# nagadomi/nunif

Hardware: AMD Instinct MI355X
Metric: input MPix/s, waifu2x swin_unet 2x tiled render (tile 256) of 1080p frames (higher is better)
Workload: dtype f16; 1 GPU; waifu2x swin_unet 2x (art scale2x geometry), tile_size=256, 1080p frame, random-init weights; tile_size=256, tile_batch=45, tiles_per_frame=45, concurrent_streams=2, parallelism=frame-sharded x1

## Files before the change

include/nunif_hip.h:

```cpp
#ifndef NUNIF_HIP_H
#define NUNIF_HIP_H

#include <stddef.h>
#include <stdint.h>

#ifdef __cplusplus
extern "C" {
#endif

#define NUNIF_HIP_ABI_VERSION 1

typedef enum {
    NUNIF_HIP_OK = 0,
    NUNIF_HIP_EINVAL = -1,
    NUNIF_HIP_ENOMEM = -2,
    NUNIF_HIP_EHIP = -3,
    NUNIF_HIP_EMISSING = -4,
    NUNIF_HIP_EUNSUPPORTED = -5
} nunif_hip_status;

int nunif_hip_abi_version(void);
const char *nunif_hip_last_error(void);

typedef struct {
    int32_t x_h, x_w, scale, offset, tile_size, blend_size;
    int32_t y_h, y_w, h_blocks, w_blocks;
    int32_t pad_l, pad_r, pad_t, pad_b, y_buffer_h, y_buffer_w;
    int32_t input_tile_step, output_tile_step;
    int32_t out_tile_size;
} nunif_tile_grid;

int nunif_hip_tile_grid_init(int32_t x_h, int32_t x_w, int32_t scale, int32_t offset, int32_t tile_size,
                             int32_t blend_size, nunif_tile_grid *grid);

int nunif_hip_blend_ramp(int32_t blend_size, float *ramp );

int nunif_hip_gather_tiles(const float *x, float *tiles, const nunif_tile_grid *grid, int32_t channels,
                           int32_t tile_begin, int32_t n_tiles, void *stream);

int nunif_hip_stitch_tiles(const float *tile_out, float *y, const nunif_tile_grid *grid, int32_t channels,
                           void *stream);

typedef struct {
    const char *name;
    const float *data;
    int32_t ndim;
    int64_t shape[4];
} nunif_tensor_desc;

typedef struct nunif_swin_unet nunif_swin_unet;

int nunif_hip_swin_unet_create(const nunif_tensor_desc *tensors, int32_t n_tensors, int32_t scale_factor,
                               nunif_swin_unet **handle);
void nunif_hip_swin_unet_destroy(nunif_swin_unet *handle);

int nunif_hip_swin_unet_forward(nunif_swin_unet *handle, const float *x, float *z, int32_t batch,
                                int32_t tile_size, void *stream);

int nunif_hip_swin_unet_render(nunif_swin_unet *handle, const float *x, float *y, int32_t x_h, int32_t x_w,
                               int32_t tile_size, int32_t batch_size, void *stream);

int nunif_hip_swin_unet_render_tile_rows(nunif_swin_unet *handle, const float *x, int32_t x_h, int32_t x_w,
                                         int32_t tile_size, int32_t batch_size, int32_t row_begin, int32_t row_end,
                                         void *stream);
int nunif_hip_swin_unet_tile_row_band(nunif_swin_unet *handle, int32_t x_h, int32_t x_w, int32_t tile_size,
                                      int32_t tile_row, int32_t row0, int32_t n_rows, float *band, int32_t import_band,
                                      void *stream);
int nunif_hip_swin_unet_stitch_rows(nunif_swin_unet *handle, float *y_band, int32_t x_h, int32_t x_w, int32_t tile_size,
                                    int32_t y_row_begin, int32_t y_row_end, void *stream);

typedef struct nunif_swin_unet_v2 nunif_swin_unet_v2;
int nunif_hip_swin_unet_v2_create(const nunif_tensor_desc *tensors, int32_t n_tensors, int32_t scale_factor,
                                  nunif_swin_unet_v2 **handle);
void nunif_hip_swin_unet_v2_destroy(nunif_swin_unet_v2 *handle);
int nunif_hip_swin_unet_v2_forward(nunif_swin_unet_v2 *handle, const float *x, float *z, int32_t batch, int32_t tile_size,
                                   int32_t clamp01, void *stream);

typedef struct nunif_cunet nunif_cunet;
int nunif_hip_cunet_create(const nunif_tensor_desc *tensors, int32_t n_tensors, int32_t no_clip, nunif_cunet **handle);
void nunif_hip_cunet_destroy(nunif_cunet *handle);
int nunif_hip_cunet_forward(nunif_cunet *handle, const float *x, float *z, int32_t batch, int32_t tile_size,
                            void *stream);
int nunif_hip_cunet_render(nunif_cunet *handle, const float *x, float *y, int32_t x_h, int32_t x_w,
                           int32_t tile_size, int32_t batch_size, void *stream);

int nunif_hip_tta_view(const float *x, float *y, int32_t C, int32_t H, int32_t W, int32_t view, void *stream);
int nunif_hip_tta_merge(const float *const *views, float *out, int32_t C, int32_t H, int32_t W, void *stream);
int nunif_hip_alpha_border_padding(const float *rgb, const float *alpha, float *out, float *work, int32_t H, int32_t W,
                                   int32_t offset, void *stream);

typedef struct {
    int32_t B, H, W;
    double divergence;
    double convergence;
    int32_t fill;
    int32_t synthetic_view;
    int32_t width_base;
    const float *convergence_dev;
} nunif_forward_warp_params;

int nunif_hip_forward_warp(const float *c, const float *depth, float *left, float *right, float *lmask,
                           float *rmask, const nunif_forward_warp_params *params, void *stream);

typedef struct nunif_depth_anything nunif_depth_anything;
int nunif_hip_depth_anything_create(const nunif_tensor_desc *tensors, int32_t n_tensors, nunif_depth_anything **handle);
int nunif_hip_depth_anything_create_ex(const nunif_tensor_desc *tensors, int32_t n_tensors, const int32_t *taps, float max_depth,
                                       nunif_depth_anything **handle);
void nunif_hip_depth_anything_destroy(nunif_depth_anything *handle);
int nunif_hip_depth_anything_forward(nunif_depth_anything *handle, const float *x, const float *pos, float *depth,
                                     int32_t B, int32_t h, int32_t w, void *stream);
int nunif_hip_depth_anything_reset_state(nunif_depth_anything *handle);
int nunif_hip_depth_anything_is_temporal(const nunif_depth_anything *handle);

typedef struct nunif_depth_aa nunif_depth_aa;
int nunif_hip_depth_aa_create(const nunif_tensor_desc *tensors, int32_t n_tensors, nunif_depth_aa **handle);
void nunif_hip_depth_aa_destroy(nunif_depth_aa *handle);
int nunif_hip_depth_aa_forward(nunif_depth_aa *handle, const float *x, float *y, int32_t B, int32_t h, int32_t w,
                               int32_t mode, void *stream);

typedef struct nunif_row_flow nunif_row_flow;
int nunif_hip_row_flow_create(const nunif_tensor_desc *tensors, int32_t n_tensors, nunif_row_flow **handle);
void nunif_hip_row_flow_destroy(nunif_row_flow *handle);
int nunif_hip_row_flow_delta(nunif_row_flow *handle, const float *x, float *delta, int32_t B, int32_t h, int32_t w,
                             int32_t flip, void *stream);

int nunif_hip_delta_warp(const float *c, const float *delta, float *out, int32_t B, int32_t C, int32_t H, int32_t W,
                         int32_t dh, int32_t dw, double delta_scale, int32_t flip, void *stream);

typedef struct nunif_light_inpaint nunif_light_inpaint;
int nunif_hip_light_inpaint_create(const nunif_tensor_desc *tensors, int32_t n_tensors, nunif_light_inpaint **handle);
void nunif_hip_light_inpaint_destroy(nunif_light_inpaint *handle);
int nunif_hip_light_inpaint_infer(nunif_light_inpaint *handle, const float *x, const uint8_t *mask, float *out, int32_t B,
                                  int32_t H, int32_t W, int32_t closing, int32_t inner_iter, int32_t outer_iter, void *stream);
int nunif_hip_light_inpaint_infer_ex(nunif_light_inpaint *handle, const float *x, const uint8_t *mask, float *out, int32_t B,
                                     int32_t H, int32_t W, int32_t closing, int32_t inner_iter, int32_t outer_iter,
                                     int32_t mirror_x, void *stream);

int nunif_hip_anaglyph(const float *left, const float *right, float *out, int32_t H, int32_t W, int32_t mode, void *stream);
int nunif_hip_equirectangular(const float *c, float *out, int32_t C, int32_t h, int32_t w, void *stream);

typedef struct nunif_mlbw nunif_mlbw;
int nunif_hip_mlbw_create(const nunif_tensor_desc *tensors, int32_t n_tensors, nunif_mlbw **handle);
void nunif_hip_mlbw_destroy(nunif_mlbw *handle);
int32_t nunif_hip_mlbw_num_layers(const nunif_mlbw *handle);
int nunif_hip_mlbw_delta(nunif_mlbw *handle, const float *x, float *delta, float *weight, int32_t B, int32_t h, int32_t w,
                         int32_t flip, void *stream);
int32_t nunif_hip_mlbw_has_hole_mask(const nunif_mlbw *handle);
int nunif_hip_mlbw_delta_mask(nunif_mlbw *handle, const float *x, float *delta, float *weight, float *mask_logits, int32_t B,
                              int32_t h, int32_t w, int32_t flip, void *stream);
int nunif_hip_hole_mask_postprocess(const float *logits, uint8_t *mask, float *work, int32_t B, int32_t h, int32_t w,
                                    int32_t H, int32_t W, float threshold, int32_t inner_iter, int32_t outer_iter, float *z,
                                    int32_t C, void *stream);

int nunif_hip_delta_weight_warp(const float *c, const float *delta, const float *weight, float *out, int32_t B, int32_t C,
                                int32_t H, int32_t W, int32_t dh, int32_t dw, int32_t L, double delta_scale, int32_t flip,
                                void *stream);

int nunif_hip_backward_warp(const float *c, const float *depth, float *left, float *right, int32_t B, int32_t C,
                            int32_t H, int32_t W, int32_t dh, int32_t dw, double divergence, double convergence,
                            int32_t synthetic_view, void *stream, const float *convergence_dev);

int nunif_hip_resize_aa(const float *x, float *y, float *tmp, int64_t planes, int32_t h_in, int32_t w_in,
                        int32_t h_out, int32_t w_out, int32_t bicubic, int32_t align_corners, int32_t clamp01,
                        const float *mean3, const float *std3, void *stream);

int64_t nunif_hip_dilate_edge_work_floats(int32_t B, int32_t H, int32_t W);
int nunif_hip_dilate_edge(const float *x, float *y, float *work, int32_t B, int32_t H, int32_t W, int32_t n_x,
                          int32_t n_y, void *stream);

int nunif_hip_minmax_normalize(const float *x, float *y, float *minmax, int32_t B, int64_t n_per, void *stream);

int nunif_hip_minmax(const float *x, float *minmax_keys, int32_t B, int64_t n_per, void *stream);
int nunif_hip_ema_scaler_push(float *state, const float *minmax_keys, int32_t ring_size, int64_t count, int32_t filled,
                              int32_t first, double decay, void *stream);
int nunif_hip_ema_scaler_ring_minmax(float *state, int32_t ring_size, void *stream);
int nunif_hip_range_normalize(const float *x, float *y, const float *lohi, int64_t n, int32_t max_mode, void *stream);

int nunif_hip_make_input_planes(const float *depth, float *out, int32_t B, int32_t H, int32_t W, double divergence_value,
                                double convergence_value, int32_t border_pix, void *stream, const float *convergence_dev);

int nunif_hip_stack(const void *const *srcs, int32_t n, int64_t bytes_each, void *dst, void *stream);

int nunif_hip_mask_morphology(const float *in, float *out, float *work, int32_t B, int32_t H, int32_t W, int32_t op,
                              int32_t n_a, int32_t n_b, void *stream);

int nunif_hip_reflection_pad2d(const float *x, float *y, int64_t planes, int32_t H, int32_t W, int32_t left, int32_t right,
                               int32_t top, int32_t bottom, void *stream);
int nunif_hip_depth_postprocess(const float *x, float *y, int64_t n, float max_dist, int32_t to_disparity, float eps,
                                int32_t negate, void *stream);

int nunif_hip_frame_to_tensor(const void *frame, float *chw, int32_t H, int32_t W, int32_t bits, void *stream);
int nunif_hip_stereo_to_frame(const float *left, const float *right, void *frame, int32_t H, int32_t W,
                              int32_t layout, int32_t bits, void *stream);
int nunif_hip_stereo_compose(const float *left, const float *right, float *out, int32_t H, int32_t W,
                             int32_t layout, void *stream);

int nunif_hip_rgb_noise(float *out, int32_t planes, int32_t H, int32_t W, int32_t level, int32_t component, uint64_t seed,
                        uint64_t counter, void *stream);
int nunif_hip_apply_rgb_noise(const float *rgb, const float *noise, float *out, int64_t n, double strength, double gamma,
                              int32_t light_decay, double light_decay_strength, void *stream);
int nunif_hip_grain_blend(float *buf, const float *noise, int64_t n, double speed, int32_t first, void *stream);
int nunif_hip_grain_video_step(const float *rgb, float *noise_buffer, void *frame, int32_t H, int32_t W, int32_t bits,
                               int32_t level, uint64_t seed, uint64_t counter, double speed, int32_t first, double strength,
                               double gamma, int32_t light_decay, double light_decay_strength, void *stream);
int nunif_hip_frame_to_tensor_rot(const void *frame, float *chw, int32_t H, int32_t W, int32_t bits, int32_t turns,
                                  void *stream);

int nunif_hip_map_depth(const float *x, float *y, int64_t n, int32_t kind, double p0, double p1, void *stream);

typedef struct nunif_transnetv2 nunif_transnetv2;
int nunif_hip_transnetv2_create(const nunif_tensor_desc *tensors, int32_t n_tensors, int32_t filters,
                                nunif_transnetv2 **handle);
void nunif_hip_transnetv2_destroy(nunif_transnetv2 *handle);
int nunif_hip_transnetv2_forward(nunif_transnetv2 *handle, const float *frames, int32_t B, int32_t T, float *one_hot,
                                 float *many_hot, float *sigmoid_out, void *stream);

typedef struct nunif_sod_v1 nunif_sod_v1;
int nunif_hip_sod_v1_create(const nunif_tensor_desc *tensors, int32_t n_tensors, int32_t net_size, nunif_sod_v1 **handle);
void nunif_hip_sod_v1_destroy(nunif_sod_v1 *handle);
int64_t nunif_hip_sod_v1_workspace_floats(int32_t B);
int nunif_hip_sod_v1_forward(nunif_sod_v1 *handle, const float *rgb, int32_t H, int32_t W, const float *depth, int32_t h,
                             int32_t w, int32_t B, float *workspace, float *saliency, float *depth_scaled, void *stream);
int nunif_hip_sod_v1_entry(const float *rgb, int32_t H, int32_t W, const float *depth, int32_t h, int32_t w, int32_t B,
                           float *x6, float *depth_scaled, void *stream);
int nunif_hip_sod_v1_debug_taps(nunif_sod_v1 *handle, const float *workspace, int32_t B, const char *name, float *out,
                                int64_t capacity, int64_t *shape4, void *stream);
int nunif_hip_sod_v1_depth_position(const float *saliency, const float *depth, int32_t B, int64_t n, double pos, float *out,
                                    void *stream);
int nunif_hip_sod_v1_ema(const float *z, float *out, int32_t B, float *state, double decay, uint64_t reset_mask, void *stream);

typedef struct nunif_superpoint nunif_superpoint;
int nunif_hip_superpoint_create(const nunif_tensor_desc *tensors, int32_t n_tensors, nunif_superpoint **handle);
void nunif_hip_superpoint_destroy(nunif_superpoint *handle);
int nunif_hip_superpoint_forward(nunif_superpoint *handle, const float *image, int32_t B, int32_t C, int32_t H, int32_t W,
                                 int32_t nms_radius, int32_t remove_borders, float threshold, float *keypoints,
                                 float *kp_scores, int32_t *counts, void *stream);
int nunif_hip_superpoint_debug_taps(nunif_superpoint *handle, const char *name, float *out, int64_t capacity, int64_t *shape4,
                                    void *stream);
int nunif_hip_superpoint_sample(nunif_superpoint *handle, int32_t b, const float *keypoints, int32_t n, float *out,
                                void *stream);

int64_t nunif_hip_superpoint_keypoints_work_floats(int32_t B, int32_t H, int32_t W);
int nunif_hip_superpoint_keypoints(const float *scores, int32_t B, int32_t H, int32_t W, int32_t nms_radius,
                                   int32_t remove_borders, float threshold, float *work, float *nms_out, float *keypoints,
                                   float *kp_scores, int32_t *counts, void *stream);

int nunif_hip_sample_descriptors(const float *keypoints, int32_t n, const float *dense, int32_t h, int32_t w, int32_t C,
                                 int32_t stride, float *out, void *stream);

int nunif_hip_superpoint_match(const float *d1, int32_t n1, const float *d2, int32_t n2, int32_t D, void *work, int64_t *index,
                               float *max_similarity, void *stream);

int nunif_hip_affine_warp(const float *x, const float *params, float *out, int32_t B, int32_t C, int32_t H, int32_t W,
                          int32_t padding_mode, void *stream);

typedef struct nunif_outpaint nunif_outpaint;
int nunif_hip_outpaint_create(const nunif_tensor_desc *tensors, int32_t n_tensors, nunif_outpaint **handle);
void nunif_hip_outpaint_destroy(nunif_outpaint *handle);
int64_t nunif_hip_outpaint_work_bytes(int32_t B, int32_t H, int32_t W, int32_t max_size);
int nunif_hip_outpaint_infer(nunif_outpaint *handle, const float *x, const uint8_t *mask, int32_t B, int32_t H, int32_t W,
                             int32_t max_size, int32_t mode, float *out, void *work, void *stream);
int nunif_hip_outpaint_debug_taps(nunif_outpaint *handle, const void *work, int32_t B, int32_t H, int32_t W, int32_t max_size,
                                  const char *name, float *out, int64_t capacity, int64_t *shape4, void *stream);
int nunif_hip_outpaint_buffer_step(const float *frames, const float *coarse, float *buffer, const uint8_t *reset,
                                   double buffer_decay, int32_t B, int32_t H, int32_t W, float *out, uint8_t *mask0,
                                   void *stream);

int nunif_hip_autocrop_stats(const float *x, int32_t B, int32_t H, int32_t W, int32_t flat, int32_t passes,
                             int32_t *border_count_tb, int32_t *border_count_lr, void *work, int64_t work_bytes, void *stream);
int nunif_hip_autocrop_debug_stats(const float *x, int32_t B, int32_t H, int32_t W, int32_t flat, int32_t passes,
                                   int32_t *border_count_tb, int32_t *border_count_lr, void *work, int64_t work_bytes,
                                   float *row_a, float *row_b, float *col_a, float *col_b, void *stream);
int nunif_hip_autocrop_crop_pad(const float *src, float *dst, int64_t N, int32_t sH, int32_t sW, int32_t dH, int32_t dW,
                                int32_t y0, int32_t x0, int32_t pad_top, int32_t pad_left, int32_t win_h, int32_t win_w,
                                float pad_value, void *stream);

int nunif_hip_jpeg_quant_tables(int32_t quality, uint8_t *luma, uint8_t *chroma);
int64_t nunif_hip_jpeg_header(int32_t H, int32_t W, int32_t quality, int32_t subsampling, int32_t restart_mcus, uint8_t *out,
                              int64_t capacity);
int64_t nunif_hip_jpeg_max_bytes(int32_t H, int32_t W, int32_t subsampling, int32_t restart_mcus);
int64_t nunif_hip_jpeg_workspace_bytes(int32_t B, int32_t H, int32_t W, int32_t subsampling, int32_t restart_mcus);
int nunif_hip_jpeg_encode(const float *rgb, int32_t B, int32_t H, int32_t W, int32_t quality, int32_t subsampling,
                          int32_t restart_mcus, uint8_t *out, int64_t capacity, int32_t *out_len, void *workspace, void *stream);
int nunif_hip_jpeg_debug_coefficients(const float *rgb, int32_t B, int32_t H, int32_t W, int32_t quality, int32_t subsampling,
                                      int16_t *coef, void *stream);

typedef struct nunif_hdr2sdr_params {
    double exposure, white_point, saturation_gain;
} nunif_hdr2sdr_params;
int nunif_hip_hdr2sdr(const void *src, void *dst, int32_t H, int32_t W, int32_t trc, int32_t colorspace,
                      const nunif_hdr2sdr_params *params, int32_t form, void *stream);
int nunif_hip_hdr2sdr_constants(int32_t trc, int32_t colorspace, const nunif_hdr2sdr_params *params, float *matrix,
                                float *hable_white);

typedef struct nunif_pixfmt_planes {
    void *data[3];
    int64_t pitch[3];
} nunif_pixfmt_planes;
int nunif_hip_yuv_to_tensor(const nunif_pixfmt_planes *src, int32_t format, int32_t H, int32_t W, int32_t matrix,
                            int32_t full_range, int32_t form, float *dst, void *frame, void *stream);
int nunif_hip_tensor_to_yuv(const float *src, int32_t H, int32_t W, int32_t format, int32_t matrix, int32_t full_range,
                            const nunif_pixfmt_planes *dst, void *stream);
int nunif_hip_pixfmt_constants(int32_t matrix, int32_t full_range, int32_t bits, int32_t direction, float *coefficients,
                               float *offsets);

typedef struct nunif_cliqa nunif_cliqa;
int nunif_hip_cliqa_create(const nunif_tensor_desc *tensors, int32_t n_tensors, int32_t kind, nunif_cliqa **handle);
void nunif_hip_cliqa_destroy(nunif_cliqa *handle);
int64_t nunif_hip_cliqa_workspace_bytes(nunif_cliqa *handle, int32_t B, int32_t H, int32_t W, int32_t group);
int nunif_hip_cliqa_forward(nunif_cliqa *handle, const float *x, int32_t B, int32_t H, int32_t W, int32_t group, void *workspace,
                            int64_t workspace_bytes, float *out0, float *out1, void *stream);
int nunif_hip_cliqa_debug_taps(nunif_cliqa *handle, const float *x, int32_t B, int32_t H, int32_t W, int32_t group,
                               void *workspace, int64_t workspace_bytes, float *out0, float *out1, void *tap1, void *tap2,
                               void *tap3, float *head_maps, void *stream);
int nunif_hip_cliqa_select_patches(const float *image, int32_t H, int32_t W, int32_t patch_size, int32_t num_patches,
                                   float *scores, int64_t *indices, float *patches, void *stream);

int64_t nunif_hip_png_header(int32_t H, int32_t W, int32_t form, const char *const *text_keys, const char *const *text_values,
                             int32_t n_text, uint8_t *out, int64_t capacity);
int64_t nunif_hip_png_max_bytes(int32_t H, int32_t W, int32_t form, int32_t stripe_rows);
int64_t nunif_hip_png_workspace_bytes(int32_t B, int32_t H, int32_t W, int32_t form, int32_t stripe_rows);
int nunif_hip_png_encode(const void *src, int32_t form, int32_t B, int32_t H, int32_t W, int32_t stripe_rows, uint8_t *out,
                         int64_t capacity, int32_t *out_len, void *workspace, void *stream);
int nunif_hip_png_debug_filtered(const void *src, int32_t form, int32_t B, int32_t H, int32_t W, uint8_t *filtered, void *stream);
int nunif_hip_png_debug_codes(const void *src, int32_t form, int32_t B, int32_t H, int32_t W, int32_t stripe_rows, int32_t *hist,
                              int32_t *lengths, void *workspace, void *stream);

int nunif_hip_swin_unet_debug_taps(nunif_swin_unet *handle, int32_t enable);
int nunif_hip_swin_unet_get_tap(nunif_swin_unet *handle, int32_t index, char *name, int32_t name_cap,
                                void *host_dst, int64_t cap_bytes, int64_t *nbytes);
int nunif_hip_cunet_debug_taps(nunif_cunet *handle, int32_t enable);
int nunif_hip_cunet_get_tap(nunif_cunet *handle, int32_t index, char *name, int32_t name_cap,
                            void *host_dst, int64_t cap_bytes, int64_t *nbytes);

int nunif_hip_profile_enable(int32_t on);
typedef struct { char name[48]; double total_ms; int64_t launches; double flops; double bytes; } nunif_prof_record;
int nunif_hip_profile_read(nunif_prof_record *out, int32_t cap, int32_t reset);

#ifdef __cplusplus
}
#endif
#endif
```

nunif_amd/_hip.py:

```python
import ctypes
import os

_HERE = os.path.dirname(os.path.abspath(__file__))
LIB_PATH = os.environ.get("NUNIF_HIP_LIB") or os.path.join(_HERE, "libnunif_hip.so")

c_void_p, c_int32, c_int64, c_float, c_char_p, c_double, c_uint64 = (
    ctypes.c_void_p, ctypes.c_int32, ctypes.c_int64, ctypes.c_float, ctypes.c_char_p, ctypes.c_double, ctypes.c_uint64)


class NunifHipError(RuntimeError):
    def __init__(self, status, message):
        super().__init__(f"libnunif_hip error {status}: {message}")
        self.status = status


class TileGrid(ctypes.Structure):
    _fields_ = [(n, c_int32) for n in (
        "x_h", "x_w", "scale", "offset", "tile_size", "blend_size",
        "y_h", "y_w", "h_blocks", "w_blocks",
        "pad_l", "pad_r", "pad_t", "pad_b", "y_buffer_h", "y_buffer_w",
        "input_tile_step", "output_tile_step", "out_tile_size")]

    def as_config(self):
        return {"y_h": self.y_h, "y_w": self.y_w, "h_blocks": self.h_blocks, "w_blocks": self.w_blocks,
                "pad": (self.pad_l, self.pad_r, self.pad_t, self.pad_b),
                "y_buffer_h": self.y_buffer_h, "y_buffer_w": self.y_buffer_w,
                "input_tile_step": self.input_tile_step, "output_tile_step": self.output_tile_step}


class TensorDesc(ctypes.Structure):
    _fields_ = [("name", c_char_p), ("data", c_void_p), ("ndim", c_int32), ("shape", c_int64 * 4)]


class ForwardWarpParams(ctypes.Structure):
    _fields_ = [("B", c_int32), ("H", c_int32), ("W", c_int32), ("divergence", c_double), ("convergence", c_double),
                ("fill", c_int32), ("synthetic_view", c_int32), ("width_base", c_int32), ("convergence_dev", c_void_p)]


class Hdr2SdrParams(ctypes.Structure):
    _fields_ = [("exposure", c_double), ("white_point", c_double), ("saturation_gain", c_double)]


class PixfmtPlanes(ctypes.Structure):
    _fields_ = [("data", c_void_p * 3), ("pitch", c_int64 * 3)]


class ProfRecord(ctypes.Structure):
    _fields_ = [("name", ctypes.c_char * 48), ("total_ms", c_double), ("launches", c_int64),
                ("flops", c_double), ("bytes", c_double)]


SIGNATURES = {
    "nunif_hip_abi_version": (c_int32, []),
    "nunif_hip_last_error": (c_char_p, []),
    "nunif_hip_tile_grid_init": (c_int32, [c_int32] * 6 + [ctypes.POINTER(TileGrid)]),
    "nunif_hip_blend_ramp": (c_int32, [c_int32, ctypes.POINTER(c_float)]),
    "nunif_hip_gather_tiles": (c_int32, [c_void_p, c_void_p, ctypes.POINTER(TileGrid), c_int32, c_int32, c_int32, c_void_p]),
    "nunif_hip_stitch_tiles": (c_int32, [c_void_p, c_void_p, ctypes.POINTER(TileGrid), c_int32, c_void_p]),
    "nunif_hip_swin_unet_create": (c_int32, [ctypes.POINTER(TensorDesc), c_int32, c_int32, ctypes.POINTER(c_void_p)]),
    "nunif_hip_swin_unet_destroy": (None, [c_void_p]),
    "nunif_hip_swin_unet_forward": (c_int32, [c_void_p, c_void_p, c_void_p, c_int32, c_int32, c_void_p]),
    "nunif_hip_swin_unet_render": (c_int32, [c_void_p, c_void_p, c_void_p, c_int32, c_int32, c_int32, c_int32, c_void_p]),
    "nunif_hip_swin_unet_render_tile_rows": (c_int32, [c_void_p, c_void_p, c_int32, c_int32, c_int32, c_int32, c_int32, c_int32, c_void_p]),
    "nunif_hip_swin_unet_tile_row_band": (c_int32, [c_void_p, c_int32, c_int32, c_int32, c_int32, c_int32, c_int32, c_void_p, c_int32, c_void_p]),
    "nunif_hip_swin_unet_stitch_rows": (c_int32, [c_void_p, c_void_p, c_int32, c_int32, c_int32, c_int32, c_int32, c_void_p]),
    "nunif_hip_swin_unet_v2_create": (c_int32, [ctypes.POINTER(TensorDesc), c_int32, c_int32, ctypes.POINTER(c_void_p)]),
    "nunif_hip_swin_unet_v2_destroy": (None, [c_void_p]),
    "nunif_hip_swin_unet_v2_forward": (c_int32, [c_void_p, c_void_p, c_void_p, c_int32, c_int32, c_int32, c_void_p]),
    "nunif_hip_cunet_create": (c_int32, [ctypes.POINTER(TensorDesc), c_int32, c_int32, ctypes.POINTER(c_void_p)]),
    "nunif_hip_cunet_destroy": (None, [c_void_p]),
    "nunif_hip_cunet_forward": (c_int32, [c_void_p, c_void_p, c_void_p, c_int32, c_int32, c_void_p]),
    "nunif_hip_cunet_render": (c_int32, [c_void_p, c_void_p, c_void_p, c_int32, c_int32, c_int32, c_int32, c_void_p]),
    "nunif_hip_forward_warp": (c_int32, [c_void_p, c_void_p, c_void_p, c_void_p, c_void_p, c_void_p,
                                         ctypes.POINTER(ForwardWarpParams), c_void_p]),
    "nunif_hip_backward_warp": (c_int32, [c_void_p, c_void_p, c_void_p, c_void_p] + [c_int32] * 6 +
                                [c_double, c_double, c_int32, c_void_p, c_void_p]),
    "nunif_hip_row_flow_create": (c_int32, [ctypes.POINTER(TensorDesc), c_int32, ctypes.POINTER(c_void_p)]),
    "nunif_hip_row_flow_destroy": (None, [c_void_p]),
    "nunif_hip_row_flow_delta": (c_int32, [c_void_p, c_void_p, c_void_p, c_int32, c_int32, c_int32, c_int32, c_void_p]),
    "nunif_hip_delta_warp": (c_int32, [c_void_p, c_void_p, c_void_p] + [c_int32] * 6 + [c_double, c_int32, c_void_p]),
    "nunif_hip_mlbw_create": (c_int32, [ctypes.POINTER(TensorDesc), c_int32, ctypes.POINTER(c_void_p)]),
    "nunif_hip_mlbw_destroy": (None, [c_void_p]),
    "nunif_hip_mlbw_num_layers": (c_int32, [c_void_p]),
    "nunif_hip_mlbw_delta": (c_int32, [c_void_p, c_void_p, c_void_p, c_void_p, c_int32, c_int32, c_int32, c_int32, c_void_p]),
    "nunif_hip_light_inpaint_create": (c_int32, [ctypes.POINTER(TensorDesc), c_int32, ctypes.POINTER(c_void_p)]),
    "nunif_hip_light_inpaint_destroy": (None, [c_void_p]),
    "nunif_hip_light_inpaint_infer": (c_int32, [c_void_p, c_void_p, c_void_p, c_void_p] + [c_int32] * 6 + [c_void_p]),
    "nunif_hip_light_inpaint_infer_ex": (c_int32, [c_void_p, c_void_p, c_void_p, c_void_p] + [c_int32] * 7 + [c_void_p]),
    "nunif_hip_anaglyph": (c_int32, [c_void_p, c_void_p, c_void_p, c_int32, c_int32, c_int32, c_void_p]),
    "nunif_hip_equirectangular": (c_int32, [c_void_p, c_void_p, c_int32, c_int32, c_int32, c_void_p]),
    "nunif_hip_mlbw_has_hole_mask": (c_int32, [c_void_p]),
    "nunif_hip_mlbw_delta_mask": (c_int32, [c_void_p, c_void_p, c_void_p, c_void_p, c_void_p, c_int32, c_int32, c_int32, c_int32,
                                            c_void_p]),
    "nunif_hip_hole_mask_postprocess": (c_int32, [c_void_p, c_void_p, c_void_p] + [c_int32] * 5 + [c_float, c_int32, c_int32,
                                                  c_void_p, c_int32, c_void_p]),
    "nunif_hip_delta_weight_warp": (c_int32, [c_void_p, c_void_p, c_void_p, c_void_p] + [c_int32] * 7 +
                                    [c_double, c_int32, c_void_p]),
    "nunif_hip_depth_aa_create": (c_int32, [ctypes.POINTER(TensorDesc), c_int32, ctypes.POINTER(c_void_p)]),
    "nunif_hip_depth_aa_destroy": (None, [c_void_p]),
    "nunif_hip_depth_aa_forward": (c_int32, [c_void_p, c_void_p, c_void_p, c_int32, c_int32, c_int32, c_int32, c_void_p]),
    "nunif_hip_depth_anything_create": (c_int32, [ctypes.POINTER(TensorDesc), c_int32, ctypes.POINTER(c_void_p)]),
    "nunif_hip_depth_anything_create_ex": (c_int32, [ctypes.POINTER(TensorDesc), c_int32, ctypes.POINTER(c_int32), ctypes.c_float,
                                                     ctypes.POINTER(c_void_p)]),
    "nunif_hip_depth_anything_destroy": (None, [c_void_p]),
    "nunif_hip_depth_anything_forward": (c_int32, [c_void_p, c_void_p, c_void_p, c_void_p, c_int32, c_int32, c_int32, c_void_p]),
    "nunif_hip_depth_anything_reset_state": (c_int32, [c_void_p]),
    "nunif_hip_depth_anything_is_temporal": (c_int32, [c_void_p]),
    "nunif_hip_tta_view": (c_int32, [c_void_p, c_void_p, c_int32, c_int32, c_int32, c_int32, c_void_p]),
    "nunif_hip_tta_merge": (c_int32, [ctypes.POINTER(c_void_p), c_void_p, c_int32, c_int32, c_int32, c_void_p]),
    "nunif_hip_alpha_border_padding": (c_int32, [c_void_p, c_void_p, c_void_p, c_void_p, c_int32, c_int32, c_int32, c_void_p]),
    "nunif_hip_resize_aa": (c_int32, [c_void_p, c_void_p, c_void_p, c_int64] + [c_int32] * 7 +
                            [ctypes.POINTER(c_float), ctypes.POINTER(c_float), c_void_p]),
    "nunif_hip_dilate_edge": (c_int32, [c_void_p, c_void_p, c_void_p] + [c_int32] * 5 + [c_void_p]),
    "nunif_hip_dilate_edge_work_floats": (ctypes.c_int64, [c_int32, c_int32, c_int32]),
    "nunif_hip_minmax_normalize": (c_int32, [c_void_p, c_void_p, c_void_p, c_int32, c_int64, c_void_p]),
    "nunif_hip_mask_morphology": (c_int32, [c_void_p, c_void_p, c_void_p] + [c_int32] * 6 + [c_void_p]),
    "nunif_hip_reflection_pad2d": (c_int32, [c_void_p, c_void_p, c_int64, c_int32, c_int32, c_int32, c_int32, c_int32, c_int32,
                                             c_void_p]),
    "nunif_hip_depth_postprocess": (c_int32, [c_void_p, c_void_p, c_int64, c_float, c_int32, c_float, c_int32, c_void_p]),
    "nunif_hip_frame_to_tensor": (c_int32, [c_void_p, c_void_p, c_int32, c_int32, c_int32, c_void_p]),
    "nunif_hip_stereo_to_frame": (c_int32, [c_void_p, c_void_p, c_void_p, c_int32, c_int32, c_int32, c_int32, c_void_p]),
    "nunif_hip_stereo_compose": (c_int32, [c_void_p, c_void_p, c_void_p, c_int32, c_int32, c_int32, c_void_p]),
    "nunif_hip_rgb_noise": (c_int32, [c_void_p, c_int32, c_int32, c_int32, c_int32, c_int32, c_uint64, c_uint64, c_void_p]),
    "nunif_hip_apply_rgb_noise": (c_int32, [c_void_p, c_void_p, c_void_p, c_int64, c_double, c_double, c_int32, c_double, c_void_p]),
    "nunif_hip_grain_blend": (c_int32, [c_void_p, c_void_p, c_int64, c_double, c_int32, c_void_p]),
    "nunif_hip_grain_video_step": (c_int32, [c_void_p, c_void_p, c_void_p, c_int32, c_int32, c_int32, c_int32, c_uint64, c_uint64,
                                             c_double, c_int32, c_double, c_double, c_int32, c_double, c_void_p]),
    "nunif_hip_frame_to_tensor_rot": (c_int32, [c_void_p, c_void_p, c_int32, c_int32, c_int32, c_int32, c_void_p]),
    "nunif_hip_map_depth": (c_int32, [c_void_p, c_void_p, c_int64, c_int32, c_double, c_double, c_void_p]),
    "nunif_hip_transnetv2_create": (c_int32, [ctypes.POINTER(TensorDesc), c_int32, c_int32, ctypes.POINTER(c_void_p)]),
    "nunif_hip_transnetv2_destroy": (None, [c_void_p]),
    "nunif_hip_transnetv2_forward": (c_int32, [c_void_p, c_void_p, c_int32, c_int32, c_void_p, c_void_p, c_void_p, c_void_p]),
    "nunif_hip_sod_v1_create": (c_int32, [ctypes.POINTER(TensorDesc), c_int32, c_int32, ctypes.POINTER(c_void_p)]),
    "nunif_hip_sod_v1_destroy": (None, [c_void_p]),
    "nunif_hip_sod_v1_workspace_floats": (c_int64, [c_int32]),
    "nunif_hip_sod_v1_forward": (c_int32, [c_void_p, c_void_p, c_int32, c_int32, c_void_p, c_int32, c_int32, c_int32, c_void_p,
                                           c_void_p, c_void_p, c_void_p]),
    "nunif_hip_sod_v1_entry": (c_int32, [c_void_p, c_int32, c_int32, c_void_p, c_int32, c_int32, c_int32, c_void_p, c_void_p,
                                         c_void_p]),
    "nunif_hip_sod_v1_debug_taps": (c_int32, [c_void_p, c_void_p, c_int32, c_char_p, c_void_p, c_int64, ctypes.POINTER(c_int64),
                                              c_void_p]),
    "nunif_hip_sod_v1_depth_position": (c_int32, [c_void_p, c_void_p, c_int32, c_int64, c_double, c_void_p, c_void_p]),
    "nunif_hip_sod_v1_ema": (c_int32, [c_void_p, c_void_p, c_int32, c_void_p, c_double, c_uint64, c_void_p]),
    "nunif_hip_superpoint_create": (c_int32, [ctypes.POINTER(TensorDesc), c_int32, ctypes.POINTER(c_void_p)]),
    "nunif_hip_superpoint_destroy": (None, [c_void_p]),
    "nunif_hip_superpoint_forward": (c_int32, [c_void_p, c_void_p] + [c_int32] * 6 + [c_float, c_void_p, c_void_p, c_void_p,
                                              c_void_p]),
    "nunif_hip_superpoint_debug_taps": (c_int32, [c_void_p, c_char_p, c_void_p, c_int64, ctypes.POINTER(c_int64), c_void_p]),
    "nunif_hip_superpoint_sample": (c_int32, [c_void_p, c_int32, c_void_p, c_int32, c_void_p, c_void_p]),
    "nunif_hip_superpoint_keypoints_work_floats": (c_int64, [c_int32, c_int32, c_int32]),
    "nunif_hip_superpoint_keypoints": (c_int32, [c_void_p] + [c_int32] * 5 + [c_float] + [c_void_p] * 6),
    "nunif_hip_sample_descriptors": (c_int32, [c_void_p, c_int32, c_void_p] + [c_int32] * 4 + [c_void_p, c_void_p]),
    "nunif_hip_superpoint_match": (c_int32, [c_void_p, c_int32, c_void_p, c_int32, c_int32, c_void_p, c_void_p, c_void_p,
                                            c_void_p]),
    "nunif_hip_affine_warp": (c_int32, [c_void_p, c_void_p, c_void_p] + [c_int32] * 5 + [c_void_p]),
    "nunif_hip_outpaint_create": (c_int32, [ctypes.POINTER(TensorDesc), c_int32, ctypes.POINTER(c_void_p)]),
    "nunif_hip_outpaint_destroy": (None, [c_void_p]),
    "nunif_hip_outpaint_work_bytes": (c_int64, [c_int32] * 4),
    "nunif_hip_outpaint_infer": (c_int32, [c_void_p, c_void_p, c_void_p] + [c_int32] * 5 + [c_void_p, c_void_p, c_void_p]),
    "nunif_hip_outpaint_debug_taps": (c_int32, [c_void_p, c_void_p] + [c_int32] * 4 + [c_char_p, c_void_p, c_int64,
                                                ctypes.POINTER(c_int64), c_void_p]),
    "nunif_hip_outpaint_buffer_step": (c_int32, [c_void_p] * 4 + [c_double] + [c_int32] * 3 + [c_void_p] * 3),
    "nunif_hip_autocrop_stats": (c_int32, [c_void_p] + [c_int32] * 5 + [c_void_p, c_void_p, c_void_p, c_int64, c_void_p]),
    "nunif_hip_autocrop_debug_stats": (c_int32, [c_void_p] + [c_int32] * 5 + [c_void_p, c_void_p, c_void_p, c_int64] +
                                       [c_void_p] * 5),
    "nunif_hip_autocrop_crop_pad": (c_int32, [c_void_p, c_void_p, c_int64] + [c_int32] * 10 + [c_float, c_void_p]),
    "nunif_hip_jpeg_quant_tables": (c_int32, [c_int32, c_void_p, c_void_p]),
    "nunif_hip_jpeg_header": (c_int64, [c_int32] * 5 + [c_void_p, c_int64]),
    "nunif_hip_jpeg_max_bytes": (c_int64, [c_int32] * 4),
    "nunif_hip_jpeg_workspace_bytes": (c_int64, [c_int32] * 5),
    "nunif_hip_jpeg_encode": (c_int32, [c_void_p] + [c_int32] * 6 + [c_void_p, c_int64, c_void_p, c_void_p, c_void_p]),
    "nunif_hip_jpeg_debug_coefficients": (c_int32, [c_void_p] + [c_int32] * 5 + [c_void_p, c_void_p]),
    "nunif_hip_png_header": (c_int64, [c_int32] * 3 + [c_void_p, c_void_p, c_int32, c_void_p, c_int64]),
    "nunif_hip_png_max_bytes": (c_int64, [c_int32] * 4),
    "nunif_hip_png_workspace_bytes": (c_int64, [c_int32] * 5),
    "nunif_hip_png_encode": (c_int32, [c_void_p] + [c_int32] * 5 + [c_void_p, c_int64, c_void_p, c_void_p, c_void_p]),
    "nunif_hip_png_debug_filtered": (c_int32, [c_void_p] + [c_int32] * 4 + [c_void_p, c_void_p]),
    "nunif_hip_png_debug_codes": (c_int32, [c_void_p] + [c_int32] * 5 + [c_void_p] * 4),
    "nunif_hip_hdr2sdr": (c_int32, [c_void_p, c_void_p, c_int32, c_int32, c_int32, c_int32, ctypes.POINTER(Hdr2SdrParams), c_int32,
                                    c_void_p]),
    "nunif_hip_hdr2sdr_constants": (c_int32, [c_int32, c_int32, ctypes.POINTER(Hdr2SdrParams), ctypes.POINTER(c_float),
                                              ctypes.POINTER(c_float)]),
    "nunif_hip_yuv_to_tensor": (c_int32, [ctypes.POINTER(PixfmtPlanes)] + [c_int32] * 6 + [c_void_p, c_void_p, c_void_p]),
    "nunif_hip_tensor_to_yuv": (c_int32, [c_void_p] + [c_int32] * 5 + [ctypes.POINTER(PixfmtPlanes), c_void_p]),
    "nunif_hip_pixfmt_constants": (c_int32, [c_int32] * 4 + [ctypes.POINTER(c_float), ctypes.POINTER(c_float)]),
    "nunif_hip_cliqa_create": (c_int32, [ctypes.POINTER(TensorDesc), c_int32, c_int32, ctypes.POINTER(c_void_p)]),
    "nunif_hip_cliqa_destroy": (None, [c_void_p]),
    "nunif_hip_cliqa_workspace_bytes": (c_int64, [c_void_p] + [c_int32] * 4),
    "nunif_hip_cliqa_forward": (c_int32, [c_void_p, c_void_p] + [c_int32] * 4 + [c_void_p, c_int64] + [c_void_p] * 3),
    "nunif_hip_cliqa_debug_taps": (c_int32, [c_void_p, c_void_p] + [c_int32] * 4 + [c_void_p, c_int64] + [c_void_p] * 7),
    "nunif_hip_cliqa_select_patches": (c_int32, [c_void_p] + [c_int32] * 4 + [c_void_p] * 4),
    "nunif_hip_swin_unet_debug_taps":(c_int32, [c_void_p, c_int32]),
    "nunif_hip_swin_unet_get_tap": (c_int32, [c_void_p, c_int32, c_char_p, c_int32, c_void_p, c_int64,
                                              ctypes.POINTER(c_int64)]),
    "nunif_hip_cunet_debug_taps": (c_int32, [c_void_p, c_int32]),
    "nunif_hip_cunet_get_tap": (c_int32, [c_void_p, c_int32, c_char_p, c_int32, c_void_p, c_int64,
                                          ctypes.POINTER(c_int64)]),
    "nunif_hip_minmax": (c_int32, [c_void_p, c_void_p, c_int32, c_int64, c_void_p]),
    "nunif_hip_ema_scaler_push": (c_int32, [c_void_p, c_void_p, c_int32, c_int64, c_int32, c_int32, c_double, c_void_p]),
    "nunif_hip_ema_scaler_ring_minmax": (c_int32, [c_void_p, c_int32, c_void_p]),
    "nunif_hip_range_normalize": (c_int32, [c_void_p, c_void_p, c_void_p, c_int64, c_int32, c_void_p]),
    "nunif_hip_make_input_planes": (c_int32, [c_void_p, c_void_p, c_int32, c_int32, c_int32, c_double, c_double, c_int32, c_void_p, c_void_p]),
    "nunif_hip_stack": (c_int32, [ctypes.POINTER(c_void_p), c_int32, c_int64, c_void_p, c_void_p]),
    "nunif_hip_profile_enable": (c_int32, [c_int32]),
    "nunif_hip_profile_read": (c_int32, [ctypes.POINTER(ProfRecord), c_int32, c_int32]),
}

_lib = None


def lib():
    global _lib
    if _lib is None:
        import torch
        if not os.path.exists(LIB_PATH):
            raise RuntimeError(
                f"{LIB_PATH} not found: the HIP engine is not built. Run `python -m nunif_amd.build` "
                "(there is no CPU fallback).")
        handle = ctypes.CDLL(LIB_PATH)
        for name, (restype, argtypes) in SIGNATURES.items():
            fn = getattr(handle, name)
            fn.restype = restype
            fn.argtypes = argtypes
        _lib = handle
    return _lib


def check(status):
    if status != 0:
        raise NunifHipError(status, lib().nunif_hip_last_error().decode("utf-8", "replace"))


def current_stream_ptr(device=None):
    import torch
    return c_void_p(torch.cuda.current_stream(device).cuda_stream)


def tile_grid(x_h, x_w, scale, offset, tile_size, blend_size):
    g = TileGrid()
    check(lib().nunif_hip_tile_grid_init(x_h, x_w, scale, offset, tile_size, blend_size or 0, ctypes.byref(g)))
    return g


def blend_ramp(blend_size):
    buf = (c_float * max(1, blend_size))()
    check(lib().nunif_hip_blend_ramp(blend_size, buf))
    return list(buf)[:blend_size]


def profile_enable(on=True):
    check(lib().nunif_hip_profile_enable(1 if on else 0))


def profile_read(reset=True):
    recs = (ProfRecord * 64)()
    n = lib().nunif_hip_profile_read(recs, 64, 1 if reset else 0)
    return [{"name": recs[i].name.decode(), "total_ms": recs[i].total_ms, "launches": recs[i].launches,
             "flops": recs[i].flops, "bytes": recs[i].bytes} for i in range(n)]
```

nunif_amd/csrc/swin_block_tail.hip:

```cpp
#include <algorithm>
#include <cstdlib>
#include <cstring>
#include <type_traits>

#include "swin_gelu.h"
#include "swin_kernels.h"

namespace nunif {

template <int C, int MF, int WAVES, bool PF = false, bool WM = false, bool G32 = false>
__global__ void __launch_bounds__(WAVES * 64)
proj_mlp_r_kernel(const f16 *__restrict__ att, f16 *x, const f16 *__restrict__ wstream, const float *__restrict__ bp,
                  const float *__restrict__ b0, const float *__restrict__ b3, long M, TailToImage ti, int rev, WinMap wm) {
    constexpr int KS = C / 32, NT = C / 16, SH = 2 * C / 32;
    constexpr int NF = 2 * KS * KS + SH * (2 * KS + NT);
    extern __shared__ __attribute__((aligned(16))) unsigned char smem_t[];
    f16x8 *wl = reinterpret_cast<f16x8 *>(smem_t);
    float *bl = reinterpret_cast<float *>(wl + (NF + KS) * 64);

    const int tid = threadIdx.x;
    const int lane = tid & 63;
    const int wave = tid >> 6;
    const int r16 = lane & 15;
    const int grp = lane >> 4;
    {
        const f16x8 *src = reinterpret_cast<const f16x8 *>(wstream);
        for (int i = tid; i < NF * 64; i += WAVES * 64) wl[i] = src[i];
        for (int i = tid; i < C; i += WAVES * 64) { bl[i] = bp[i]; bl[3 * C + i] = b3[i]; }
        for (int i = tid; i < 2 * C; i += WAVES * 64) bl[C + i] = b0[i];
        if (ti.w) {
            for (int i = tid; i < KS * 64; i += WAVES * 64) wl[NF * 64 + i] = reinterpret_cast<const f16x8 *>(ti.w)[i];
            if (tid < 16) bl[4 * C + tid] = tid < ti.n_real ? ti.bias[tid] : 0.f;
        }
    }
    __syncthreads();
    const f16x8 *wlane = wl + lane;
    auto wfrag = [&](int fi) -> f16x8 { return wlane[fi * 64]; };
    f16x8 ie, io, je, jo;
#pragma unroll
    for (int j = 0; j < 8; ++j) {
        ie[j] = (f16)((r16 == 8 * grp + j) ? 1.f : 0.f);
        io[j] = (f16)((r16 + 16 == 8 * grp + j) ? 1.f : 0.f);
        je[j] = (f16)((j < 4 && r16 == 4 * grp + j) ? 1.f : 0.f);
        jo[j] = (f16)((j >= 4 && r16 == 4 * grp + j - 4) ? 1.f : 0.f);
    }

    const long n_groups = (M + MF * 16 - 1) / (MF * 16);
    const long gstride = (long)gridDim.x * WAVES;
    auto gmap = [&](long g) { return rev ? n_groups - 1 - g : g; };
    auto token_of = [&](long g, int f) -> long {
        const long m = gmap(g) * (MF * 16) + f * 16 + r16;
        return m < M ? m : M - 1;
    };
    auto load_pixmap = [&](long g, int (&pm)[MF]) {
#pragma unroll
        for (int f = 0; f < MF; ++f) pm[f] = wm.pixmap[(int)token_of(g, f)];
    };
    auto load_group = [&](long g, const int (&pm)[MF], f16x8 (&of)[MF][KS], f16x8 (&xr)[MF][KS], long (&pixn)[MF]) {
#pragma unroll
        for (int f = 0; f < MF; ++f) {
            const long r = token_of(g, f);
            const f16 *p;
            if constexpr (WM) {
                const int ri = (int)r, w = ri / 36;
                pixn[f] = pm[f];
                p = att + (ri * 16 + w * 2880 + (grp >> 1) * 576 + 8 * (grp & 1));
            } else {
                pixn[f] = r;
                p = att + r * C + grp * 8;
            }
            const f16 *px = x + pixn[f] * C + grp * 8;
#pragma unroll
            for (int ks = 0; ks < KS; ++ks) {
                of[f][ks] = *reinterpret_cast<const f16x8 *>(p + (WM ? ks * (2 * 36 * 16) : ks * 32));
                xr[f][ks] = *reinterpret_cast<const f16x8 *>(px + ks * 32);
            }
        }
    };
    f16x8 ofn[PF ? MF : 1][PF ? KS : 1];
    f16x8 xrn[PF ? MF : 1][PF ? KS : 1];
    long pixnn[MF];
    const long g_first = (long)blockIdx.x * WAVES + wave;
    int pm_next[MF] = {};
    auto g_clamp = [&](long g) { return g < n_groups ? g : n_groups - 1; };
    if constexpr (PF) {
        if (g_first < n_groups) {
            if constexpr (WM) load_pixmap(g_first, pm_next);
            load_group(g_first, pm_next, ofn, xrn, pixnn);
            if constexpr (WM) load_pixmap(g_clamp(g_first + gstride), pm_next);
        }
    }
#pragma unroll 1
    for (long g = g_first; g < n_groups; g += gstride) {
        const long m_base = gmap(g) * (MF * 16);
        int lofs = 0;
        asm volatile("" : "+v"(lofs));
        const float *lbp = bl + lofs, *lb0 = bl + C + lofs, *lb3 = bl + 3 * C + lofs;
        long row[MF];
        bool valid[MF];
        f16x8 yf[MF][KS];
        {
            f16x8 of[MF][KS];
            f16x8 xr[MF][KS];
#pragma unroll
            for (int f = 0; f < MF; ++f) {
                const long m = m_base + f * 16 + r16;
                valid[f] = m < M;
            }
            if constexpr (PF) {
#pragma unroll
                for (int f = 0; f < MF; ++f) {
                    row[f] = pixnn[f];
#pragma unroll
                    for (int ks = 0; ks < KS; ++ks) { of[f][ks] = ofn[f][ks]; xr[f][ks] = xrn[f][ks]; }
                }
                load_group(g_clamp(g + gstride), pm_next, ofn, xrn, pixnn);
                if constexpr (WM) load_pixmap(g_clamp(g + 2 * gstride), pm_next);
            } else {
                if constexpr (WM) load_pixmap(g, pm_next);
                load_group(g, pm_next, of, xr, row);
            }
#pragma unroll
            for (int s = 0; s < KS; ++s) {
                const int n0 = 32 * s + 4 * grp;
                const f32x4 ba = *reinterpret_cast<const f32x4 *>(lbp + n0);
                const f32x4 bb = *reinterpret_cast<const f32x4 *>(lbp + n0 + 16);
                f32x4 a0[MF], a1[MF];
#pragma unroll
                for (int f = 0; f < MF; ++f) { a0[f] = ba; a1[f] = bb; }
#pragma unroll
                for (int ks = 0; ks < KS; ++ks) {
                    const f16x8 wa = wfrag((s * KS + ks) * 2);
                    const f16x8 wb = wfrag((s * KS + ks) * 2 + 1);
#pragma unroll
                    for (int f = 0; f < MF; ++f) {
                        a0[f] = MFMA_16x16x32(wa, of[f][ks], a0[f]);
                        a1[f] = MFMA_16x16x32(wb, of[f][ks], a1[f]);
                    }
                }
#pragma unroll
                for (int f = 0; f < MF; ++f) {
                    a0[f] = MFMA_16x16x32(ie, xr[f][s], a0[f]);
                    a1[f] = MFMA_16x16x32(io, xr[f][s], a1[f]);
                }
#pragma unroll
                for (int f = 0; f < MF; ++f)
                    yf[f][s] = (f16x8){(f16)a0[f][0], (f16)a0[f][1], (f16)a0[f][2], (f16)a0[f][3],
                                       (f16)a1[f][0], (f16)a1[f][1], (f16)a1[f][2], (f16)a1[f][3]};
            }
        }
        f32x4 acc[NT][MF];
#pragma unroll
        for (int s = 0; s < KS; ++s) {
            const int n0 = 32 * s + 4 * grp;
            const f32x4 ca = *reinterpret_cast<const f32x4 *>(lb3 + n0);
            const f32x4 cb = *reinterpret_cast<const f32x4 *>(lb3 + n0 + 16);
#pragma unroll
            for (int f = 0; f < MF; ++f) {
                acc[2 * s][f] = MFMA_16x16x32(je, yf[f][s], ca);
                acc[2 * s + 1][f] = MFMA_16x16x32(jo, yf[f][s], cb);
            }
        }
        constexpr int F_MLP = 2 * KS * KS;
        constexpr int F_STEP = 2 * KS + NT;
#pragma unroll 1
        for (int s = 0; s < SH; ++s) {
            const int n0 = 32 * s + 4 * grp;
            const f32x4 ba = *reinterpret_cast<const f32x4 *>(lb0 + n0);
            const f32x4 bb = *reinterpret_cast<const f32x4 *>(lb0 + n0 + 16);
            f32x4 h0[MF], h1[MF];
#pragma unroll
            for (int f = 0; f < MF; ++f) { h0[f] = ba; h1[f] = bb; }
            const f16x8 *wf = wlane + (F_MLP + s * F_STEP) * 64;
#pragma unroll
            for (int ks = 0; ks < KS; ++ks) {
                const f16x8 wa = wf[(ks * 2) * 64];
                const f16x8 wb = wf[(ks * 2 + 1) * 64];
#pragma unroll
                for (int f = 0; f < MF; ++f) {
                    h0[f] = MFMA_16x16x32(wa, yf[f][ks], h0[f]);
                    h1[f] = MFMA_16x16x32(wb, yf[f][ks], h1[f]);
                }
            }
            f16x8 hf[MF];
#pragma unroll
            for (int f = 0; f < MF; ++f) {
                hf[f] = gelu8t<G32>(h0[f], h1[f]);
            }
#pragma unroll
            for (int nt = 0; nt < NT; ++nt) {
                const f16x8 wv = wf[(2 * KS + nt) * 64];
#pragma unroll
                for (int f = 0; f < MF; ++f) acc[nt][f] = MFMA_16x16x32(wv, hf[f], acc[nt][f]);
            }
        }
        if (ti.w) {
            const int s2 = ti.ps * ti.ps;
            const f32x4 tb = *reinterpret_cast<const f32x4 *>(bl + 4 * C + 4 * grp);
#pragma unroll
            for (int f = 0; f < MF; ++f) {
                f32x4 img = tb;
#pragma unroll
                for (int ks = 0; ks < KS; ++ks) {
                    const f16x8 bfrag = {(f16)acc[2 * ks][f][0], (f16)acc[2 * ks][f][1], (f16)acc[2 * ks][f][2], (f16)acc[2 * ks][f][3],
                                         (f16)acc[2 * ks + 1][f][0], (f16)acc[2 * ks + 1][f][1], (f16)acc[2 * ks + 1][f][2],
                                         (f16)acc[2 * ks + 1][f][3]};
                    img = MFMA_16x16x32(wlane[(NF + ks) * 64], bfrag, img);
                }
                if (!valid[f]) continue;
                using pix_t = std::conditional_t<WM, unsigned, long>;
                const pix_t m = (pix_t)row[f];
                const int px = (int)(m % (pix_t)ti.W);
                const pix_t t2 = m / (pix_t)ti.W;
                const int py = (int)(t2 % (pix_t)ti.H), pb = (int)(t2 / (pix_t)ti.H);
                const int OC = ti.n_real / s2;
                const long OH = (long)ti.H * ti.ps, OW = (long)ti.W * ti.ps;
#pragma unroll
                for (int r = 0; r < 4; ++r) {
                    const int n = 4 * grp + r;
                    if (n < ti.n_real) {
                        const int c = n / s2, rem = n - c * s2, i = rem / ti.ps, j = rem - i * ti.ps;
                        ti.out[(((long)pb * OC + c) * OH + (long)py * ti.ps + i) * OW + (long)px * ti.ps + j] =
                            fminf(fmaxf(img[r], 0.f), 1.f);
                    }
                }
            }
            continue;
        }
#pragma unroll
        for (int p = 0; p < NT / 2; ++p) {
#pragma unroll
            for (int f = 0; f < MF; ++f) {
                const f16x4 oa = {(f16)acc[2 * p][f][0], (f16)acc[2 * p][f][1], (f16)acc[2 * p][f][2], (f16)acc[2 * p][f][3]};
                const f16x4 ob = {(f16)acc[2 * p + 1][f][0], (f16)acc[2 * p + 1][f][1], (f16)acc[2 * p + 1][f][2],
                                  (f16)acc[2 * p + 1][f][3]};
                const f16x8 o = pair_to_run(oa, ob);
                if (valid[f]) *reinterpret_cast<f16x8 *>(x + row[f] * C + 32 * p + pair_run_channel(grp)) = o;
            }
        }
    }
}

__global__ void winmap_build_kernel(int *__restrict__ pixmap, int B, int H, int W, int shift) {
    const int n = blockIdx.x * blockDim.x + threadIdx.x;
    const int nwx = W / 6, nwy = H / 6;
    if (n >= B * H * W) return;
    const int w = n / 36, t = n - 36 * w;
    const int wx = w % nwx, t2 = w / nwx;
    const int wy = t2 % nwy, b = t2 / nwy;
    const int iy = t / 6, ix = t - 6 * iy;
    int yy = wy * 6 + iy + shift, xx = wx * 6 + ix + shift;
    if (yy >= H) yy -= H;
    if (xx >= W) xx -= W;
    pixmap[n] = (b * H + yy) * W + xx;
}

int launch_winmap_build(int *pixmap, int B, int H, int W, int shift, hipStream_t s) {
    NUNIF_REQUIRE(H % 6 == 0 && W % 6 == 0 && (long)B * H * W < (1L << 31), "winmap: geometry %d x %d x %d", B, H, W);
    const long n = (long)B * H * W;
    if (n == 0) return NUNIF_HIP_OK;
    winmap_build_kernel<<<(unsigned)((n + 255) / 256), 256, 0, s>>>(pixmap, B, H, W, shift);
    NUNIF_LAUNCH_CHECK();
    return NUNIF_HIP_OK;
}

constexpr int proj_mlp_stream_frags_c(int C) { return 2 * (C / 32) * (C / 32) + (2 * C / 32) * (2 * (C / 32) + C / 16); }

int proj_mlp_stream_frags(int C) {
    const int KS = C / 32, NT = C / 16, SH = 2 * C / 32;
    return 2 * KS * KS + SH * (2 * KS + NT);
}

int launch_proj_mlp(const f16 *att, f16 *x, const f16 *wstream, const float *bp, const float *b0, const float *b3,
                    long M, int C, hipStream_t s, const TailToImage *to_image, int rev, const WinMap *wmap, int gelu32) {
    if (M == 0) return NUNIF_HIP_OK;
    NUNIF_REQUIRE(C == 96, "proj_mlp: channel count %d unsupported (C = 192 runs launch_proj_mlp_ws)", C);
    NUNIF_REQUIRE(!to_image || to_image->n_real <= 16, "proj_mlp: the fused image head takes at most 16 output channels");
    ProfScope ps("proj_mlp_r_kernel<96,2,8,true>", s, 2.0 * (double)M * C * C * 5.0, (double)M * C * 2.0 * 3.0);
    constexpr size_t smem = (size_t)(proj_mlp_stream_frags_c(96) + 3) * 1024 + (4 * 96 + 16) * 4;
    TailToImage ti;
    memset(&ti, 0, sizeof(ti));
    if (to_image) ti = *to_image;
    WinMap wm;
    memset(&wm, 0, sizeof(wm));
    if (wmap) wm = *wmap;
    NUNIF_REQUIRE(!wm.on || (wm.pixmap && wm.H % 6 == 0 && wm.W % 6 == 0 && M % ((long)wm.H * wm.W) == 0 && 96L * M < (1L << 31)),
                  "proj_mlp: window map geometry");
    constexpr int MF = 2, WAVES = 8;
    auto go = [&](auto kern, int slot) -> int {
        static bool configured[4] = {false, false, false, false};
        if (!configured[slot]) {
            NUNIF_HIP_CHECK(hipFuncSetAttribute((const void *)kern, hipFuncAttributeMaxDynamicSharedMemorySize, (int)smem));
            configured[slot] = true;
        }
        const long groups = (M + MF * 16 - 1) / (MF * 16);
        const unsigned blocks = (unsigned)std::min<long>((groups + WAVES - 1) / WAVES, 256);
        kern<<<blocks, WAVES * 64, smem, s>>>(att, x, wstream, bp, b0, b3, M, ti, rev, wm);
        return NUNIF_HIP_OK;
    };
    int rc;
    if (gelu32) rc = wm.on ? go(proj_mlp_r_kernel<96, MF, WAVES, true, true, true>, 3) : go(proj_mlp_r_kernel<96, MF, WAVES, true, false, true>, 2);
    else rc = wm.on ? go(proj_mlp_r_kernel<96, MF, WAVES, true, true, false>, 1) : go(proj_mlp_r_kernel<96, MF, WAVES, true, false, false>, 0);
    if (rc) return rc;
    NUNIF_LAUNCH_CHECK();
    return NUNIF_HIP_OK;
}

}
```

nunif_amd/csrc/swin_kernels.h:

```cpp
#pragma once
#include "common.h"

namespace nunif {

struct GemmArgs {
    const f16 *a; int B, Hi, Wi, Cin;
    int Ho, Wo, stride, oy, ox, kw;
    int K;
    const f16 *w;
    const float *bias;
    int N;
    int mode;
    int act;
    float slope;
    const f16 *res;
    void *out;
    int ldo;
    int n_real;
    int ps;
    int oshift, OH, OW;
    int no_clamp;
    int lda;
    int rev;
    int nt_chunk;
    int res_H = 0, res_W = 0, res_crop = 0;
    const float *in_scale = nullptr;
};
int launch_gemm(const GemmArgs &g, hipStream_t s, const char *tag);

struct PatchUpArgs { const f16 *a, *w; const float *bias; const f16 *res; f16 *out; int B, Ho, Wo, Cq, rev; };
bool patchup_supported(const PatchUpArgs &g);
int launch_patchup(const PatchUpArgs &g, hipStream_t s);

struct PatchDownArgs { const f16 *a, *w; const float *bias; f16 *out; int B, Ho, Wo, Cin, oy, rev; int N = 192; int act = 0; float slope = 0.f; };
bool patchdown_supported(const PatchDownArgs &g);
int launch_patchdown(const PatchDownArgs &g, hipStream_t s);

struct CunetUpArgs { const f16 *a, *w; const float *bias; const f16 *res; f16 *out; const float *in_scale; int B, S, res_S, crop;
                     float slope; };
bool cunet_up_supported(const CunetUpArgs &g);
int launch_cunet_up(const CunetUpArgs &g, hipStream_t s);

struct GemmOsArgs {
    const f16 *a; long M; int lda, K;
    const f16 *w; const float *bias; int N;
    int act;
    const f16 *res;
    f16 *out; int ldo;
    float2 *stats_out;
    const float2 *stats_in; int stats_parts; const float *wsum; float ln_eps;
};
bool gemm_os_supported(long M, int N, int K);
bool gemm_os_consumes_stats(long M, int N, int K);
int launch_gemm_os(const GemmOsArgs &g, hipStream_t s, const char *tag);

struct DaMlpArgs {
    f16 *t; long M;
    const f16 *w1; const float *b1, *ws1;
    const f16 *w2c; const float *b2;
    const float2 *stats_in; float2 *stats_out; float ln_eps;
    void *partial; unsigned *flags;
};
bool da_mlp_supported(int D, int hidden);

struct CunetHeadArgs { const f16 *a, *w; const float *bias; float *out32; const float *add32; int B, Hi, Wi, Ho, Wo, addH, addW, add_crop, clamp01; };
bool cunet_head_supported(const CunetHeadArgs &g);
int launch_cunet_head(const CunetHeadArgs &g, hipStream_t s);

constexpr int kVdaGnBlocks = 256;
int launch_vda_groupnorm(const f16 *x, const float *gamma, const float *beta, f16 *y, float2 *part, int frames, int P, int C, float eps, hipStream_t s);
int launch_vda_layernorm(const f16 *x, const float *gamma, const float *beta, f16 *y, long T, int C, float eps, hipStream_t s);
int launch_vda_geglu(const f16 *h, f16 *out, long T, int I, hipStream_t s);
struct VdaTattnArgs { const f16 *qkv; f16 *kc, *vc; const float *pq, *pk, *pv; f16 *att; int P, C, hd, start, idx; };
int launch_vda_tattn(const VdaTattnArgs &g, hipStream_t s);
long da_mlp_partial_bytes(long M);
long da_mlp_flag_count(long M);
int launch_da_mlp(const DaMlpArgs &a, hipStream_t s);

struct Stem1Args {
    const float *x;
    int frame_mode, H, W, wb, istep, pad_t, pad_l, tile_begin;
    int B, T;
    const float *w;
    const float *bias;
    int C1, C1P;
    f16 *out;
    float slope;
};
int launch_stem1(const Stem1Args &a, hipStream_t s);

struct StemFusedArgs {
    const float *x;
    int frame_mode, H, W, wb, istep, pad_t, pad_l, tile_begin;
    int B, T;
    const f16 *w1;
    const f16 *w2;
    const float *b2;
    f16 *out;
    float slope;
    int rev;
    int C1, C, crop;
};
bool stem_fused_supported(int C1, int C);
int launch_stem_fused(const StemFusedArgs &a, hipStream_t s);

int proj_mlp_stream_frags(int C);
struct TailToImage { const f16 *w; const float *bias; float *out; int H, W, ps, n_real; };
struct WinMap { int on, H, W, shift; const int *pixmap; };
int launch_winmap_build(int *pixmap, int B, int H, int W, int shift, hipStream_t s);
int launch_proj_mlp(const f16 *att, f16 *x, const f16 *wstream, const float *bp, const float *b0, const float *b3,
                    long M, int C, hipStream_t s, const TailToImage *to_image = nullptr, int rev = 0,
                    const WinMap *wm = nullptr, int gelu32 = 0);

int swin_block96_tail_frags();
int swin_block96_btab_floats();
int launch_swin_block96(f16 *x, const f16 *wqkv, const float *bqkv, const float *btab, const f16 *wtail, const float *bp,
                        const float *b0, const float *b3, int B, int H, int W, int shift, hipStream_t s,
                        const TailToImage *ti = nullptr, int rev = 0);

int proj_mlp_ws_stream_frags();
int launch_proj_mlp_ws(const f16 *att, f16 *x, const f16 *wws, const float *bp, const float *b0, const float *b3, long M,
                       hipStream_t s, int rev = 0, int gelu32 = 0);

constexpr int kQkvBiasFloatsPerHead = 36 * 52;
int launch_qkv_attn_r(const f16 *x, f16 *att, const f16 *wres, const float *bqkv, const float *btab32,
                      int B, int H, int W, int C, int heads, int shift, hipStream_t s, int rev = 0, int window_major = 0);

int launch_window_attn(const f16 *qkv, f16 *out, const float *bias, int B, int H, int W, int heads, int hd,
                       int shift, hipStream_t s);

int launch_layernorm_nobias(const f16 *x, f16 *y, const float *gamma, long M, int C, hipStream_t s);

struct ConvArgs {
    const f16 *a; const f16 *a2;
    int H2, W2, crop2;
    int B, Hi, Wi, Cin, Ho, Wo, stride, kh, kw;
    const f16 *wstream;
    const float *bias;
    int N, n_real;
    int act; float slope;
    f16 *out;
    float *out32;
    const float *add32; int addH, addW, add_crop;
    int clamp01;
    int rpad;
    const f16 *res;
    int zpad;
    int relu_in;
    const f16 *res2;
    int ldo;
    int cmaj;
    float *part32;
};
long gemm_big_m();
int launch_conv(const ConvArgs &g, hipStream_t s);
bool conv3_lds_applies(const ConvArgs &g);
int launch_conv3_lds(const ConvArgs &g, hipStream_t s);
bool conv3_dma_applies(const ConvArgs &g);
int launch_conv3_dma(const ConvArgs &g, hipStream_t s);

struct C3ConvArgs {
    const float *x; int frame_mode, H, W, wb, istep, pad_t, pad_l, tile_begin;
    int B, T;
    const float *w, *bias;
    int C;
    f16 *out;
    float slope;
};
int launch_c3_conv(const C3ConvArgs &a, hipStream_t s);

int launch_se(f16 *x, float *sums, float *scale, const float *w1, const float *b1, const float *w2, const float *b2,
              int B, long hw, int C, hipStream_t s, int scale_in_consumer = 0);

}
```

nunif_amd/csrc/swin_qkv_attn_r.hip:

```cpp
#include <algorithm>
#include <cstdlib>

#include "swin_kernels.h"

namespace nunif {


constexpr float kRegionR = 100.0f;

struct QkvAttnRArgs {
    const f16 *x;
    f16 *att;
    const f16 *wres;
    const float *bqkv;
    const float *btab32;
    int B, H, W, shift, n_windows;
    int rev;
};

__device__ __forceinline__ f16x4 mul4_to_f16(const f32x4 &o, float inv) {
    return (f16x4){(f16)__builtin_fmaf(o[0], inv, 0.0f), (f16)__builtin_fmaf(o[1], inv, 0.0f), (f16)__builtin_fmaf(o[2], inv, 0.0f),
                   (f16)__builtin_fmaf(o[3], inv, 0.0f)};
}
__device__ __forceinline__ f16x4 lone_to_f16x4(float e, float zf) {
    return (f16x4){(f16)e, (f16)zf, (f16)0.f, (f16)0.f};
}

constexpr int kBiasStride = 52;


__device__ __host__ inline int win_token(int mt, int r16) { return mt < 2 ? 16 * mt + r16 : ((r16 & 3) == 0 ? 32 + (r16 >> 2) : 35); }

template <int C, int HD, int HPP, int WAVES = 8, bool WM = false>
__global__ void __launch_bounds__(WAVES * 64)
qkv_attn_r_kernel(QkvAttnRArgs a) {
    constexpr int kWavesR = WAVES;
    constexpr int NTHR = WAVES * 64;
    constexpr int KS = C / 32;
    constexpr int HEADS = C / HD;
    constexpr int NTH = HD / 16;
    constexpr int FPH = 3 * NTH * KS;
    constexpr int PASSES = HEADS / HPP;
    static_assert(HEADS == 6 && HEADS % HPP == 0, "swin_unet uses 6 heads at every level");
    extern __shared__ __attribute__((aligned(16))) unsigned char smem_r[];
    f16x8 *wl = reinterpret_cast<f16x8 *>(smem_r);
    float *bt32 = reinterpret_cast<float *>(wl + HPP * FPH * 64);
    float *bl = bt32 + HPP * kQkvBiasFloatsPerHead;

    const int tid = threadIdx.x;
    const int lane = tid & 63;
    const int wave = __builtin_amdgcn_readfirstlane(tid >> 6);
    const int r16 = lane & 15;
    const int grp = lane >> 4;
    const int nwx = a.W / 6, nwy = a.H / 6;
    const f16x4 zero4 = {(f16)0.f, (f16)0.f, (f16)0.f, (f16)0.f};
    float zf = 0.f;
    asm("" : "+s"(zf));

    for (int i = tid; i < 3 * C; i += NTHR) bl[i] = a.bqkv[i];
    const f16x8 ones8 = {(f16)1.f, (f16)1.f, (f16)1.f, (f16)1.f, (f16)1.f, (f16)1.f, (f16)1.f, (f16)1.f};

    int tokc[3];
#pragma unroll
    for (int mt = 0; mt < 3; ++mt) tokc[mt] = win_token(mt, r16);
    unsigned wm_off[3];
#pragma unroll
    for (int mt = 0; mt < 3; ++mt) wm_off[mt] = (unsigned)((tokc[mt] * HD + 4 * grp) * 2);
    const bool store2 = (r16 & 3) == 0;
    const int st_delta = (NTH == 2 ? pair_run_channel(grp) : 4 * grp) * 2 - 16 * grp;
    f16x4 rk0 = zero4, rq0 = zero4;
    if (a.shift > 0 && grp == 2) { rk0[0] = (f16)1.f; rq0[0] = (f16)kRegionR; }

    const int n_wg = gridDim.x / PASSES;
    const int wstride = kWavesR * n_wg;
    const bool spread = a.n_windows < 8 * wstride;
    const int w0 = spread ? wave * n_wg + (int)(blockIdx.x / PASSES) : (int)(blockIdx.x / PASSES) * kWavesR + wave;
    const int pass = blockIdx.x % PASSES;
    {
        const f16x8 *src = reinterpret_cast<const f16x8 *>(a.wres) + (long)pass * HPP * FPH * 64;
        for (int i = tid; i < HPP * FPH * 64; i += NTHR) wl[i] = src[i];
        const f32x4 *bsrc = reinterpret_cast<const f32x4 *>(a.btab32 + (long)pass * HPP * kQkvBiasFloatsPerHead);
        for (int i = tid; i < HPP * kQkvBiasFloatsPerHead / 4; i += NTHR) reinterpret_cast<f32x4 *>(bt32)[i] = bsrc[i];
    }
    __syncthreads();

    int cx = w0 % nwx, cy = (w0 / nwx) % nwy, cb = w0 / (nwx * nwy);
    const int dx = wstride % nwx, dy = (wstride / nwx) % nwy, db = wstride / (nwx * nwy);
    const long img_bytes = (long)a.H * a.W * C * 2;

    auto load_x = [&](int wb, int wy, int wx, bool special, f16x8 (&xf)[3][KS], unsigned (&vo)[3]) {
        const int y0 = wy * 6 + a.shift, x0 = wx * 6 + a.shift;
        const char *xb = reinterpret_cast<const char *>(a.x) + (long)wb * img_bytes;
        if (special) {
#pragma unroll
            for (int mt = 0; mt < 3; ++mt) {
                const int tk = win_token(mt, r16), iy = tk / 6, ix = tk - 6 * iy;
                int yy = y0 + iy, xx = x0 + ix;
                if (yy >= a.H) yy -= a.H;
                if (xx >= a.W) xx -= a.W;
                vo[mt] = (unsigned)(((yy * a.W + xx) * C + 8 * grp) * 2);
            }
        } else {
            const unsigned org = (unsigned)((y0 * a.W + x0) * C * 2);
            int rl = r16;
            asm("" : "+v"(rl));
#pragma unroll
            for (int mt = 0; mt < 3; ++mt) {
                const int tk = win_token(mt, rl), iy = (tk * 43) >> 8, ix = tk - 6 * iy;
                vo[mt] = org + (unsigned)(((iy * a.W + ix) * C + 8 * grp) * 2);
            }
        }
#pragma unroll
        for (int mt = 0; mt < 3; ++mt) {
#pragma unroll
            for (int ks = 0; ks < KS; ++ks) xf[mt][ks] = *reinterpret_cast<const f16x8 *>(xb + vo[mt] + 64 * ks);
        }
    };
    auto decode = [&](int &wb, int &wy, int &wx, bool &special) {
        wb = a.rev ? a.B - 1 - cb : cb;
        wy = a.rev ? nwy - 1 - cy : cy;
        wx = a.rev ? nwx - 1 - cx : cx;
        special = a.shift > 0 && (wy == nwy - 1 || wx == nwx - 1);
    };
    auto advance = [&]() {
        cx += dx;
        if (cx >= nwx) { cx -= nwx; ++cy; }
        cy += dy;
        if (cy >= nwy) { cy -= nwy; ++cb; }
        cb += db;
    };

    auto qkv_bias = [&](int hl, int head, int part, int nt) -> f32x4 {
        const int ch0 = part * C + head * HD + nt * 16;
        if (part == 2) { const float bv = bl[ch0 + r16]; return (f32x4){bv, bv, bv, bv}; }
        return *reinterpret_cast<const f32x4 *>(bl + ch0 + 4 * grp);
    };
    auto bias_frag = [&](int hl, int qt, int kt) -> f32x4 {
        return *reinterpret_cast<const f32x4 *>(bt32 + (hl * 36 + tokc[qt]) * kBiasStride + 4 * grp + 16 * kt);
    };
    f16x8 xf[3][KS];
    unsigned vo[3];
    int wb, wy, wx;
    bool special;
    f16x8 wnx = wl[lane];
    auto run_windows = [&]() {
    int wi = w0;
    decode(wb, wy, wx, special);
    auto step = [&]() { advance(); wi += wstride; decode(wb, wy, wx, special); };
    if (wi < a.n_windows) load_x(wb, wy, wx, special, xf, vo);
#pragma unroll 1
    while (wi < a.n_windows) {
        const int wq = (wb * nwy + wy) * nwx + wx;
        char *ab = reinterpret_cast<char *>(a.att) + (WM ? (long)wq * (HEADS * 36 * HD * 2) : (long)wb * img_bytes);
        const unsigned wm_base = (unsigned)__builtin_amdgcn_readfirstlane((unsigned)wq * (unsigned)(HEADS * 36 * HD * 2));

        constexpr bool kEarlyX = C == 96 && WM;
        auto run_heads = [&]() {
        const bool sp_now = special;
        f16x4 rkr[3], rqr[3];
        if (special) {
            const bool last_y = wy == nwy - 1, last_x = wx == nwx - 1;
#pragma unroll
            for (int mt = 0; mt < 3; ++mt) {
                const int tk = win_token(mt, r16), iy = tk / 6, ix = tk - 6 * iy;
                const int reg = ((last_y && iy >= 3) ? 2 : 0) + ((last_x && ix >= 3) ? 1 : 0);
#pragma unroll
                for (int j = 0; j < 4; ++j) {
                    const bool on = grp == 2 && reg == j;
                    rkr[mt][j] = (f16)(on ? 1.f : 0.f);
                    rqr[mt][j] = (f16)(on ? kRegionR : 0.f);
                }
            }
        } else {
#pragma unroll
            for (int mt = 0; mt < 3; ++mt) { rkr[mt] = rk0; rqr[mt] = rq0; }
        }
        constexpr int kHeadUnroll = C == 96 ? HPP : 1;
#pragma unroll kHeadUnroll
        for (int hl = 0; hl < HPP; ++hl) {
            const int head = pass * HPP + hl;
            const f16x8 *wh = wl + (hl * FPH) * 64 + lane;
            constexpr bool kPrefetchW = C == 96;
            f16x4 qt4[NTH][3], kt4[NTH][3], vt4[NTH][3];
            f16x8 wq2[2];
            wq2[0] = kPrefetchW ? wnx : wh[0];
            f32x4 bnx = qkv_bias(hl, head, 0, 0);
#pragma unroll
            for (int part = 0; part < 3; ++part) {
#pragma unroll
                for (int nt = 0; nt < NTH; ++nt) {
                    const int fidx = (part * NTH + nt) * KS;
                    f32x4 acc[3];
                    bnx = qkv_bias(hl, head, part, nt);
#pragma unroll
                    for (int mt = 0; mt < 3; ++mt) acc[mt] = bnx;
#pragma unroll
                    for (int ks = 0; ks < KS; ++ks) {
                        const int f = fidx + ks;
                        if constexpr (kPrefetchW)
                            wq2[(f + 1) & 1] = (f + 1 < FPH) ? wh[(f + 1) * 64] : (hl + 1 < HPP ? wh[FPH * 64] : wl[lane]);
                        else wq2[f & 1] = wh[f * 64];
                        const f16x8 w = wq2[f & 1];
#pragma unroll
                        for (int mt = 0; mt < 3; ++mt)
                            acc[mt] = part == 2 ? MFMA_16x16x32(xf[mt][ks], w, acc[mt]) : MFMA_16x16x32(w, xf[mt][ks], acc[mt]);
                    }
#pragma unroll
                    for (int mt = 0; mt < 3; ++mt) {
                        const f16x4 v = {(f16)acc[mt][0], (f16)acc[mt][1], (f16)acc[mt][2], (f16)acc[mt][3]};
                        if (part == 0) qt4[nt][mt] = v; else if (part == 1) kt4[nt][mt] = v; else vt4[nt][mt] = v;
                    }
                }
            }
            if constexpr (kPrefetchW) wnx = wq2[FPH & 1];
            if constexpr (kEarlyX) {
                if (hl == HPP - 1) {
                    step();
                    if (wi < a.n_windows) load_x(wb, wy, wx, special, xf, vo);
                }
            }

#pragma unroll
            for (int qt = 0; qt < 3; ++qt) {
                f32x4 s[3];
                {
                    f32x4 sb[3];
#pragma unroll
                    for (int kt = 0; kt < 3; ++kt) sb[kt] = bias_frag(hl, qt, kt);
#pragma unroll
                    for (int kt = 0; kt < 3; ++kt) {
                        f32x4 acc = sb[kt];
                        if constexpr (HD == 16) {
                            acc = MFMA_16x16x32(cat8(kt4[0][kt], rkr[kt]), cat8(qt4[0][qt], rqr[qt]), acc);
                        } else {
                            acc = MFMA_16x16x32(cat8(kt4[0][kt], kt4[1][kt]), cat8(qt4[0][qt], qt4[1][qt]), acc);
                            if (sp_now) acc = MFMA_16x16x32(cat8(rkr[kt], zero4), cat8(rqr[qt], zero4), acc);
                        }
                        s[kt] = acc;
                    }
                }
                float mx = fmaxf(fmaxf(fmaxf(fmaxf(s[0][0], s[0][1]), s[0][2]), fmaxf(fmaxf(s[0][3], s[1][0]), s[1][1])),
                                 fmaxf(fmaxf(s[1][2], s[1][3]), s[2][0]));
                mx = row_group_max(mx);
                f16x4 pf[3];
#pragma unroll
                for (int kt = 0; kt < 2; ++kt) {
                    const float p0 = __builtin_amdgcn_exp2f(s[kt][0] - mx), p1 = __builtin_amdgcn_exp2f(s[kt][1] - mx);
                    const float p2 = __builtin_amdgcn_exp2f(s[kt][2] - mx), p3 = __builtin_amdgcn_exp2f(s[kt][3] - mx);
                    pf[kt] = (f16x4){(f16)p0, (f16)p1, (f16)p2, (f16)p3};
                }
                pf[2] = lone_to_f16x4(__builtin_amdgcn_exp2f(s[2][0] - mx), zf);
                const f16x8 psum = cat8(pf[0] + pf[1], pf[2]);
                const f32x4 z4 = {0.f, 0.f, 0.f, 0.f};
                const f32x4 sm = MFMA_16x16x32(ones8, psum, z4);
                const float inv = __builtin_amdgcn_rcpf(sm[0]);
                const bool store = qt < 2 || store2;
                f16x4 ov[NTH];
#pragma unroll
                for (int dt = 0; dt < NTH; ++dt) {
                    f32x4 o = MFMA_16x16x32(cat8(vt4[dt][0], vt4[dt][1]), cat8(pf[0], pf[1]), z4);
                    o = MFMA_16x16x32(cat8(zero4, vt4[dt][2]), psum, o);
                    ov[dt] = mul4_to_f16(o, inv);
                }
                if constexpr (NTH == 2) {
                    const f16x8 run = pair_to_run(ov[0], ov[1]);
                    if (store) *reinterpret_cast<f16x8 *>(ab + (vo[qt] + (unsigned)st_delta) + head * (HD * 2)) = run;
                } else if constexpr (WM) {
                    unsigned long hb = reinterpret_cast<unsigned long>(a.att) + (wm_base + (unsigned)(head * (36 * HD * 2)));
                    asm("" : "+s"(hb));
                    typedef __attribute__((address_space(1))) char gchar;
                    typedef __attribute__((address_space(1))) f16x4 gf16x4;
                    unsigned lo = wm_off[qt];
                    asm("" : "+v"(lo));
                    if (store) *reinterpret_cast<gf16x4 *>(reinterpret_cast<gchar *>(hb) + lo) = ov[0];
                } else {
                    if (store) *reinterpret_cast<f16x4 *>(ab + (vo[qt] + (unsigned)st_delta) + head * (HD * 2)) = ov[0];
                }
            }
            if constexpr (kHeadUnroll > 1) __builtin_amdgcn_sched_barrier(0);
        }
        };
        run_heads();

        if constexpr (!kEarlyX) {
            step();
            if (wi < a.n_windows) load_x(wb, wy, wx, special, xf, vo);
        }
    }
    };
    run_windows();
}

int qkv_attn_r_frags(int C) { return 3 * (C / 16) * (C / 32); }

template <int C, int HD, int HPP, int WAVES = 8, bool WM = false>
static int launch_r(const QkvAttnRArgs &a, int grid, hipStream_t s) {
    constexpr size_t smem = (size_t)HPP * 3 * (HD / 16) * (C / 32) * 1024 + HPP * kQkvBiasFloatsPerHead * 4 + (size_t)3 * C * 4;
    static bool configured = false;
    if (!configured) {
        NUNIF_HIP_CHECK(hipFuncSetAttribute((const void *)qkv_attn_r_kernel<C, HD, HPP, WAVES, WM>,
                                            hipFuncAttributeMaxDynamicSharedMemorySize, (int)smem));
        configured = true;
    }
    qkv_attn_r_kernel<C, HD, HPP, WAVES, WM><<<grid, WAVES * 64, smem, s>>>(a);
    return NUNIF_HIP_OK;
}

int launch_qkv_attn_r(const f16 *x, f16 *att, const f16 *wres, const float *bqkv, const float *btab32,
                      int B, int H, int W, int C, int heads, int shift, hipStream_t s, int rev, int window_major) {
    NUNIF_REQUIRE(H % 6 == 0 && W % 6 == 0, "qkv_attn: %dx%d not a multiple of the 6x6 window", H, W);
    NUNIF_REQUIRE(heads == 6 && (C == 96 || C == 192), "qkv_attn: C=%d heads=%d unsupported", C, heads);
    if (H <= 6) shift = 0;
    QkvAttnRArgs a;
    a.x = x; a.att = att; a.wres = wres; a.bqkv = bqkv; a.btab32 = btab32;
    a.B = B; a.H = H; a.W = W; a.shift = shift;
    a.n_windows = B * (H / 6) * (W / 6);
    a.rev = rev;
    NUNIF_REQUIRE(!window_major || C == 96, "qkv_attn: the window-major att map exists for C = 96 only");
    NUNIF_REQUIRE(!window_major || (long)a.n_windows * (6 * 36 * 16 * 2) < (1L << 32),
                  "qkv_attn: the window-major att map of %d windows does not fit 32-bit byte offsets", a.n_windows);
    const double tok = (double)B * H * W;
    const int kWavesR = C == 96 ? 16 : 8;
    const int wgs = (a.n_windows + kWavesR - 1) / kWavesR;
    int grid = wgs < 256 ? wgs : 256;
    if (C == 192) grid = std::max(2, grid & ~1);
    int rc;
    if (C == 96) {
        ProfScope ps("qkv_attn_r_kernel<96,16>", s, 2.0 * tok * C * 3.0 * C + 4.0 * tok * 36.0 * C, tok * C * 4.0);
        rc = window_major ? launch_r<96, 16, 6, 16, true>(a, grid, s) : launch_r<96, 16, 6, 16, false>(a, grid, s);
    } else {
        ProfScope ps("qkv_attn_r_kernel<192,32>", s, 2.0 * tok * C * 3.0 * C + 4.0 * tok * 36.0 * C, tok * C * 4.0);
        rc = launch_r<192, 32, 3>(a, grid, s);
    }
    if (rc) return rc;
    NUNIF_LAUNCH_CHECK();
    return NUNIF_HIP_OK;
}

}
```

nunif_amd/csrc/swin_unet.cpp:

```cpp
#include <algorithm>
#include <cmath>
#include <cstdlib>
#include <cstring>
#include <string>
#include <vector>

#include "host_weights.h"
#include "swin_kernels.h"

namespace nunif {

int launch_stitch(const float *tile_out, float *y, const nunif_tile_grid *g, int C, hipStream_t s, int y0 = 0, int rows = -1,
                  int compact = 0);

namespace {

struct Linear {
    f16 *w = nullptr;
    float *bias = nullptr;
    int N = 0, n_real = 0, K = 0;
};

struct Block {
    Linear qkv, proj, mlp0, mlp3;
    Linear mlp0p, mlp3p;
    float *norm1 = nullptr, *norm2 = nullptr;
    bool fast = true;
    float *attn_bias = nullptr;
    f16 *tail_stream = nullptr;
    f16 *tail_ws = nullptr;
    f16 *qkv_res = nullptr;
    float *qkv_rbias = nullptr;
    float *attn_btab32 = nullptr;
    f16 *b96_tail = nullptr;
    float *b96_btab = nullptr;
};

}
}

using namespace nunif;

struct nunif_swin_unet : DeviceOwner {
    int scale_factor = 2;
    int C = 96, heads = 6;
    int C1 = 48, C1P = 64;
    int top_dim = 96;
    float *stem1_w = nullptr, *stem1_b = nullptr;
    Linear stem2, down1, down2, up2, up1, proj2, to_image, to_image_pre;
    Linear down2b;
    bool down2_split = false;
    f16 *to_image_chained = nullptr;
    f16 *stemf_w1 = nullptr, *stemf_w2 = nullptr;
    int dir = 0;
    int att_wm = 1;
    int gelu32 = 0;
    int block96 = 0;
    bool has_proj2 = false;
    std::vector<Block> swin[5];
    DeviceBuf s1, f1, f2, f3, g1, qkv, att, hid, tile_out;
    DeviceBuf winmap[2];
    int winmap_B = 0, winmap_S = 0;
    int device = 0;
    struct Tap { std::string name; void *dev; size_t bytes; };
    bool taps_on = false;
    std::vector<Tap> taps;
    void clear_taps() { for (auto &t : taps) (void)hipFree(t.dev); taps.clear(); }
};

namespace nunif {
namespace {

int pad16(int n) { return (n + 15) / 16 * 16; }

template <typename F>
int make_linear(nunif_swin_unet *h, int n_real, int K, F wt, const float *bias, Linear *L, bool chained = false,
                std::vector<f16> *keep = nullptr) {
    const int N = pad16(n_real);
    std::vector<f16> packed = pack_nt_ks(n_real, N, K, wt, chained);
    std::vector<float> b(N, 0.0f);
    for (int n = 0; n < n_real; ++n) b[n] = bias[n];
    L->N = N; L->n_real = n_real; L->K = K;
    if (keep) *keep = packed;
    int rc = h->upload(packed, &L->w);
    if (rc) return rc;
    return h->upload(b, &L->bias);
}

int make_plain_linear(nunif_swin_unet *h, const TensorMap &m, const std::string &key, int n_real, int K, Linear *L,
                      bool chained = false, std::vector<f16> *keep = nullptr) {
    const HostTensor *w, *b;
    int rc;
    if ((rc = find(m, key + ".weight", &w)) || (rc = find(m, key + ".bias", &b))) return rc;
    NUNIF_REQUIRE(w->numel == (int64_t)n_real * K && b->numel == n_real, "%s: unexpected shape", key.c_str());
    const float *wd = w->data;
    return make_linear(h, n_real, K, [=](int n, int k) { return wd[(size_t)n * K + k]; }, b->data, L, chained, keep);
}

int make_stage(nunif_swin_unet *h, const TensorMap &m, const std::string &key, int dim, int layers,
               std::vector<Block> *blocks) {
    blocks->resize(layers);
    const int heads = h->heads;
    for (int i = 0; i < layers; ++i) {
        const std::string p = key + ".block." + std::to_string(i) + ".";
        Block &bl = (*blocks)[i];
        int rc;
        std::vector<f16> hq;
        if ((rc = make_plain_linear(h, m, p + "attn.qkv", 3 * dim, dim, &bl.qkv, false, &hq))) return rc;
        const bool has_norm = m.find(p + "norm1.weight") != m.end();
        bl.fast = heads == 6 && (dim == 96 || dim == 192) && !has_norm;
        if (has_norm) {
            const HostTensor *n1, *n2;
            if ((rc = find(m, p + "norm1.weight", &n1)) || (rc = find(m, p + "norm2.weight", &n2))) return rc;
            NUNIF_REQUIRE(n1->numel == dim && n2->numel == dim, "%snorm: shape", p.c_str());
            NUNIF_REQUIRE(m.find(p + "norm1.bias") == m.end(), "%snorm1: LayerNorm with bias is not a reference variant", p.c_str());
            std::vector<float> g1(n1->data, n1->data + dim), g2(n2->data, n2->data + dim);
            if ((rc = h->upload(g1, &bl.norm1)) || (rc = h->upload(g2, &bl.norm2))) return rc;
        }
        if (!bl.fast) {
            if ((rc = make_plain_linear(h, m, p + "attn.proj", dim, dim, &bl.proj)) ||
                (rc = make_plain_linear(h, m, p + "mlp.0", 2 * dim, dim, &bl.mlp0p)) ||
                (rc = make_plain_linear(h, m, p + "mlp.3", dim, 2 * dim, &bl.mlp3p)))
                return rc;
        }
        if (bl.fast) {
            const HostTensor *w, *b;
            if ((rc = find(m, p + "attn.qkv.weight", &w)) || (rc = find(m, p + "attn.qkv.bias", &b))) return rc;
            const float qs = (1.0f / sqrtf((float)(dim / heads))) * 1.4426950408889634f;
            const float *wd = w->data;
            std::vector<f16> hs = pack_nt_ks(3 * dim, 3 * dim, dim, [=](int n, int k) {
                return wd[(size_t)n * dim + k] * (n < dim ? qs : 1.0f); });
            const int KS = dim / 32, NTH = (dim / heads) / 16, nf = 3 * (dim / 16) * KS;
            std::vector<f16> stream((size_t)nf * 512, (f16)0.0f);
            size_t fi = 0;
            for (int hh = 0; hh < heads; ++hh)
                for (int part = 0; part < 3; ++part)
                    for (int nt = 0; nt < NTH; ++nt)
                        for (int ks = 0; ks < KS; ++ks)
                            copy_frag(hs, (size_t)(part * (dim / 16) + hh * NTH + nt) * KS + ks, stream, &fi);
            if ((rc = h->upload(stream, &bl.qkv_res))) return rc;
            std::vector<float> rb(3 * dim);
            for (int n = 0; n < 3 * dim; ++n) rb[n] = b->data[n] * (n < dim ? qs : 1.0f);
            if ((rc = h->upload(rb, &bl.qkv_rbias))) return rc;
        }
        std::vector<f16> hp, h0, h3;
        if (bl.fast) {
        if ((rc = make_plain_linear(h, m, p + "attn.proj", dim, dim, &bl.proj, false, &hp))) return rc;
        if ((rc = make_plain_linear(h, m, p + "mlp.0", 2 * dim, dim, &bl.mlp0, true, &h0))) return rc;
        if ((rc = make_plain_linear(h, m, p + "mlp.3", dim, 2 * dim, &bl.mlp3, true, &h3))) return rc;
        }
        if (bl.fast) {
            const int KS = dim / 32, NT = dim / 16, SH = 2 * dim / 32;
            const int nf = proj_mlp_stream_frags(dim);
            std::vector<f16> stream((size_t)(nf + 15) / 16 * 16 * 512, (f16)0.0f);
            size_t fi = 0;
            auto put = [&](const std::vector<f16> &src, int frag) { copy_frag(src, frag, stream, &fi); };
            for (int sx = 0; sx < KS; ++sx)
                for (int ks = 0; ks < KS; ++ks) { put(hp, (2 * sx) * KS + ks); put(hp, (2 * sx + 1) * KS + ks); }
            for (int sx = 0; sx < SH; ++sx) {
                for (int ks = 0; ks < KS; ++ks) { put(h0, (2 * sx) * KS + ks); put(h0, (2 * sx + 1) * KS + ks); }
                for (int nt = 0; nt < NT; ++nt) put(h3, nt * SH + sx);
            }
            NUNIF_REQUIRE((int)fi == nf, "internal: tail stream has %zu fragments, expected %d", fi, nf);
            if ((rc = h->upload(stream, &bl.tail_stream))) return rc;
            if (dim == 192) {
                std::vector<f16> ws((size_t)proj_mlp_ws_stream_frags() * 512, (f16)0.0f);
                size_t wi = 0;
                auto putw = [&](const std::vector<f16> &src, int frag) { copy_frag(src, frag, ws, &wi); };
                for (int w = 0; w < 4; ++w)
                    for (int nt = 0; nt < 3; ++nt)
                        for (int ks = 0; ks < KS; ++ks) putw(hp, (3 * w + nt) * KS + ks);
                for (int w = 0; w < 4; ++w)
                    for (int nt = 0; nt < 6; ++nt)
                        for (int ks = 0; ks < KS; ++ks) putw(h0, (6 * w + nt) * KS + ks);
                for (int w = 0; w < 4; ++w)
                    for (int nt = 0; nt < 3; ++nt)
                        for (int ks = 0; ks < SH; ++ks) putw(h3, (3 * w + nt) * SH + ks);
                NUNIF_REQUIRE((int)wi == proj_mlp_ws_stream_frags(), "internal: ws tail stream has %zu fragments", wi);
                if ((rc = h->upload(ws, &bl.tail_ws))) return rc;
            }
        }
        const HostTensor *tab;
        if ((rc = find(m, p + "attn.relative_position_bias_table", &tab))) return rc;
        NUNIF_REQUIRE(tab->numel == 121 * heads, "%s: bias table shape", p.c_str());
        if (bl.fast && dim == 96) {
            const HostTensor *pw;
            if ((rc = find(m, p + "attn.proj.weight", &pw))) return rc;
            const float *pd = pw->data;
            std::vector<f16> hpc = pack_nt_ks(dim, dim, dim, [=](int n, int k) { return pd[(size_t)n * dim + k]; }, true);
            const int KS = dim / 32, NT = dim / 16, SH = 2 * dim / 32;
            std::vector<f16> stream((size_t)swin_block96_tail_frags() * 512, (f16)0.0f);
            size_t fi = 0;
            auto put = [&](const std::vector<f16> &src, int frag) { copy_frag(src, frag, stream, &fi); };
            for (int sx = 0; sx < KS; ++sx)
                for (int ks = 0; ks < KS; ++ks) { put(hpc, (2 * sx) * KS + ks); put(hpc, (2 * sx + 1) * KS + ks); }
            for (int sx = 0; sx < SH; ++sx) {
                for (int ks = 0; ks < KS; ++ks) { put(h0, (2 * sx) * KS + ks); put(h0, (2 * sx + 1) * KS + ks); }
                for (int nt = 0; nt < NT; ++nt) put(h3, nt * SH + sx);
            }
            NUNIF_REQUIRE((int)fi == swin_block96_tail_frags(), "internal: block96 stream has %zu fragments", fi);
            if ((rc = h->upload(stream, &bl.b96_tail))) return rc;
            const int stride = swin_block96_btab_floats() / heads;
            std::vector<float> rt((size_t)heads * stride, -1000.0f);
            for (int hh = 0; hh < heads; ++hh) {
                for (int i2 = 0; i2 < 121; ++i2) rt[(size_t)hh * stride + i2] = tab->data[(size_t)(120 - i2) * heads + hh] * 1.4426950408889634f;
                rt[(size_t)hh * stride + 121] = rt[(size_t)hh * stride + 122] = rt[(size_t)hh * stride + 123] = 0.0f;
            }
            if ((rc = h->upload(rt, &bl.b96_btab))) return rc;
        }
        std::vector<float> bias((size_t)heads * 36 * 48);
        for (int hh = 0; hh < heads; ++hh)
            for (int q = 0; q < 36; ++q)
                for (int k = 0; k < 48; ++k) {
                    float v = -1.0e30f;
                    if (k < 36) {
                        const int idx = (q / 6 - k / 6 + 5) * 11 + (q % 6 - k % 6 + 5);
                        v = tab->data[(size_t)idx * heads + hh];
                    }
                    bias[((size_t)hh * 36 + q) * 48 + k] = v;
                }
        if ((rc = h->upload(bias, &bl.attn_bias))) return rc;
        std::vector<float> btab32((size_t)heads * 36 * 52, 0.0f);
        for (int hh = 0; hh < heads; ++hh)
            for (int q = 0; q < 36; ++q)
                for (int k = 0; k < 48; ++k) {
                    const int key = k < 32 ? k : (((k - 32) & 3) == 0 ? 32 + ((k - 32) >> 2) : -1);
                    btab32[((size_t)hh * 36 + q) * 52 + k] =
                        key >= 0 ? bias[((size_t)hh * 36 + q) * 48 + key] * 1.4426950408889634f : -1000.0f;
                }
        if ((rc = h->upload(btab32, &bl.attn_btab32))) return rc;
    }
    return NUNIF_HIP_OK;
}

int run_gemm(const Linear &L, const f16 *a, int B, int Hi, int Wi, int Cin, int Ho, int Wo, int stride, int oy,
             int ox, int kw, int mode, int act, float slope, const f16 *res, void *out, int ldo, int ps,
             hipStream_t s, const char *tag, int rev = 0) {
    GemmArgs g;
    g.a = a; g.B = B; g.Hi = Hi; g.Wi = Wi; g.Cin = Cin;
    g.Ho = Ho; g.Wo = Wo; g.stride = stride; g.oy = oy; g.ox = ox; g.kw = kw;
    g.K = L.K; g.w = L.w; g.bias = L.bias; g.N = L.N;
    g.mode = mode; g.act = act; g.slope = slope; g.res = res; g.out = out; g.ldo = ldo;
    g.n_real = L.n_real; g.ps = ps; g.oshift = 0; g.OH = 0; g.OW = 0; g.no_clamp = 0; g.lda = 0; g.nt_chunk = 0; g.rev = rev;
    return launch_gemm(g, s, tag);
}

int run_patchup(const Linear &L, const f16 *a, int B, int H, int W, int Cq, f16 *skip, hipStream_t s, const char *tag, int rev) {
    PatchUpArgs p = {a, L.w, L.bias, skip, skip, B, H, W, Cq, rev};
    if (L.K == 192 && L.n_real == 4 * Cq && patchup_supported(p)) return launch_patchup(p, s);
    return run_gemm(L, a, B, H, W, L.K, H, W, 1, 0, 0, 1, 1, 0, 0.f, skip, skip, Cq, 1, s, tag, rev);
}

int run_patchdown(const Linear &L, const f16 *a, int B, int Ho, int Wo, int Cin, int oy, f16 *out, hipStream_t s, const char *tag,
                  int rev) {
    PatchDownArgs p;
    p.a = a; p.w = L.w; p.bias = L.bias; p.out = out; p.B = B; p.Ho = Ho; p.Wo = Wo; p.Cin = Cin; p.oy = oy; p.rev = rev;
    if (L.K == 384 && L.n_real == 192 && patchdown_supported(p)) return launch_patchdown(p, s);
    return run_gemm(L, a, B, 2 * Ho, 2 * Wo, Cin, Ho, Wo, 2, oy, 0, 2, 0, 0, 0.f, nullptr, out, L.n_real, 1, s, tag, rev);
}

int run_linear(const Linear &L, const f16 *a, int B, int H, int W, int act, const f16 *res, f16 *out,
               hipStream_t s, const char *tag, int rev = 0) {
    return run_gemm(L, a, B, H, W, L.K, H, W, 1, 0, 0, 1, 0, act, 0.f, res, out, L.n_real, 1, s, tag, rev);
}

int tap(nunif_swin_unet *h, const std::string &name, const void *src, size_t bytes, hipStream_t s) {
    if (!h->taps_on) return NUNIF_HIP_OK;
    void *p = nullptr;
    NUNIF_HIP_CHECK(hipMalloc(&p, bytes));
    NUNIF_HIP_CHECK(hipMemcpyAsync(p, src, bytes, hipMemcpyDeviceToDevice, s));
    h->taps.push_back({name, p, bytes});
    return NUNIF_HIP_OK;
}

static int next_dir(nunif_swin_unet *h) {
    const int d = h->dir;
    h->dir ^= 1;
    return d;
}

int run_stage(nunif_swin_unet *h, std::vector<Block> &blocks, f16 *x, int B, int S, int dim, hipStream_t s,
              const char *name, const TailToImage *to_image = nullptr) {
    f16 *qkv = (f16 *)h->qkv.p, *att = (f16 *)h->att.p;
    const size_t tok = (size_t)B * S * S;
    int rc;
    for (size_t i = 0; i < blocks.size(); ++i) {
        Block &bl = blocks[i];
        const int shift = (i % 2 == 1) ? 3 : 0;
        const std::string tn = std::string(name) + ".b" + std::to_string(i);
        if (!bl.fast) {
            f16 *hid = (f16 *)h->hid.p;
            const f16 *xin = x;
            if (bl.norm1) {
                if ((rc = launch_layernorm_nobias(x, hid, bl.norm1, (long)tok, dim, s))) return rc;
                xin = hid;
            }
            if ((rc = run_linear(bl.qkv, xin, B, S, S, 0, nullptr, qkv, s, "gemm_qkv", next_dir(h)))) return rc;
            if ((rc = tap(h, tn + ".qkv", qkv, tok * 3 * dim * 2, s))) return rc;
            if ((rc = launch_window_attn(qkv, att, bl.attn_bias, B, S, S, h->heads, dim / h->heads, shift, s))) return rc;
            if ((rc = tap(h, tn + ".attn", att, tok * dim * 2, s))) return rc;
            if ((rc = run_linear(bl.proj, att, B, S, S, 0, x, x, s, "gemm_proj", next_dir(h)))) return rc;
            xin = x;
            if (bl.norm2) {
                if ((rc = launch_layernorm_nobias(x, att, bl.norm2, (long)tok, dim, s))) return rc;
                xin = att;
            }
            if ((rc = run_linear(bl.mlp0p, xin, B, S, S, 1, nullptr, hid, s, "gemm_mlp0", next_dir(h)))) return rc;
            if ((rc = run_linear(bl.mlp3p, hid, B, S, S, 0, x, x, s, "gemm_mlp3", next_dir(h)))) return rc;
            if ((rc = tap(h, tn + ".out", x, tok * dim * 2, s))) return rc;
            continue;
        }
        const bool last_blk = i + 1 == blocks.size();
        if (dim == 96 && bl.b96_tail && h->block96 && !h->taps_on) {
            if ((rc = launch_swin_block96(x, bl.qkv_res, bl.qkv_rbias, bl.b96_btab, bl.b96_tail, bl.proj.bias, bl.mlp0.bias,
                                          bl.mlp3.bias, B, S, S, shift, s, last_blk ? to_image : nullptr, next_dir(h))))
                return rc;
            if (last_blk && to_image) break;
            continue;
        }
        const bool att_wm = dim == 96 && h->att_wm && !h->taps_on && 96L * (long)tok < (1L << 31);
        if ((rc = launch_qkv_attn_r(x, att, bl.qkv_res, bl.qkv_rbias, bl.attn_btab32, B, S, S, dim, h->heads, shift, s, next_dir(h),
                                    att_wm ? 1 : 0)))
            return rc;
        if ((rc = tap(h, tn + ".attn", att, tok * dim * 2, s))) return rc;
        const bool last = i + 1 == blocks.size();
        if (dim == 192) {
            if ((rc = launch_proj_mlp_ws(att, x, bl.tail_ws, bl.proj.bias, bl.mlp0.bias, bl.mlp3.bias, (long)tok, s, next_dir(h), h->gelu32)))
                return rc;
        } else {
            const int eff_shift = S <= 6 ? 0 : shift;
            WinMap wmap = {att_wm ? 1 : 0, S, S, eff_shift, nullptr};
            if (att_wm) {
                if (h->winmap_S != S || B > h->winmap_B) {
                    for (int k = 0; k < 2; ++k) {
                        if ((rc = h->winmap[k].ensure(tok * sizeof(int)))) return rc;
                        if ((rc = launch_winmap_build((int *)h->winmap[k].p, B, S, S, k ? 3 : 0, s))) return rc;
                    }
                    h->winmap_B = B; h->winmap_S = S;
                }
                wmap.pixmap = (const int *)h->winmap[eff_shift ? 1 : 0].p;
            }
            if ((rc = launch_proj_mlp(att, x, bl.tail_stream, bl.proj.bias, bl.mlp0.bias, bl.mlp3.bias, (long)tok, dim, s,
                                      last ? to_image : nullptr, next_dir(h), &wmap, h->gelu32)))
                return rc;
        }
        if (last && to_image) break;
        if ((rc = tap(h, tn + ".out", x, tok * dim * 2, s))) return rc;
    }
    return NUNIF_HIP_OK;
}

int ensure_workspace(nunif_swin_unet *h, int B, int T) {
    const size_t S = T - 16, S2 = S / 2, S4 = S / 4, C = h->C;
    const size_t t1 = (size_t)B * S * S, t2 = (size_t)B * S2 * S2, t3 = (size_t)B * S4 * S4;
    const size_t top = h->top_dim;
    int rc;
    if ((rc = h->s1.ensure((size_t)B * (T - 14) * (T - 14) * h->C1P * 2))) return rc;
    if ((rc = h->f1.ensure(t1 * C * 2))) return rc;
    if ((rc = h->f2.ensure(t2 * 2 * C * 2))) return rc;
    if ((rc = h->f3.ensure(t3 * 2 * C * 2))) return rc;
    if (h->has_proj2 && (rc = h->g1.ensure(t1 * top * 2))) return rc;
    const size_t qkv_elems = std::max(t1 * 3 * std::max(C, top), t2 * 6 * C);
    if ((rc = h->qkv.ensure(qkv_elems * 2))) return rc;
    if ((rc = h->att.ensure(std::max(t1 * std::max(C, top), t2 * 2 * C) * 2))) return rc;
    if ((rc = h->hid.ensure(std::max(t1 * 2 * std::max(C, top), t2 * 4 * C) * 2))) return rc;
    return NUNIF_HIP_OK;
}

int forward_impl(nunif_swin_unet *h, const float *x, const float *frame, const nunif_tile_grid *grid,
                 int tile_begin, float *z, int B, int T, hipStream_t s) {
    const int S = T - 16, C = h->C;
    NUNIF_REQUIRE(T > 16 && S % 12 == 0 && S % 16 == 0, "tile_size %d is not valid for swin_unet", T);
    int rc;
    if ((rc = ensure_workspace(h, B, T))) return rc;
    f16 *s1 = (f16 *)h->s1.p, *f1 = (f16 *)h->f1.p, *f2 = (f16 *)h->f2.p, *f3 = (f16 *)h->f3.p;

    if (h->stemf_w2 && stem_fused_supported(h->C1, (int)C)) {
        StemFusedArgs sf;
        memset(&sf, 0, sizeof(sf));
        if (frame) {
            sf.x = frame; sf.frame_mode = 1; sf.H = grid->x_h; sf.W = grid->x_w; sf.wb = grid->w_blocks;
            sf.istep = grid->input_tile_step; sf.pad_t = grid->pad_t; sf.pad_l = grid->pad_l; sf.tile_begin = tile_begin;
        } else {
            sf.x = x;
        }
        sf.B = B; sf.T = T; sf.w1 = h->stemf_w1; sf.w2 = h->stemf_w2; sf.b2 = h->stem2.bias; sf.out = f1; sf.slope = 0.1f;
        h->dir = 1;
        if ((rc = launch_stem_fused(sf, s))) return rc;
        goto stem_done;
    }
    Stem1Args a1;
    memset(&a1, 0, sizeof(a1));
    if (frame) {
        a1.x = frame; a1.frame_mode = 1; a1.H = grid->x_h; a1.W = grid->x_w; a1.wb = grid->w_blocks;
        a1.istep = grid->input_tile_step; a1.pad_t = grid->pad_t; a1.pad_l = grid->pad_l; a1.tile_begin = tile_begin;
    } else {
        a1.x = x;
    }
    a1.B = B; a1.T = T; a1.w = h->stem1_w; a1.bias = h->stem1_b; a1.C1 = h->C1; a1.C1P = h->C1P; a1.out = s1;
    a1.slope = 0.1f;
    h->dir = 1;
    if ((rc = launch_stem1(a1, s))) return rc;
    if ((rc = run_gemm(h->stem2, s1, B, T - 14, T - 14, h->C1P, S, S, 1, 0, 0, 3, 0, 2, 0.1f, nullptr, f1, C, 1, s,
                              "gemm_stem2", next_dir(h))))
        return rc;
stem_done:
    if ((rc = tap(h, "stem", f1, (size_t)B * S * S * C * 2, s))) return rc;
    if ((rc = run_stage(h, h->swin[0], f1, B, S, C, s, "swin1"))) return rc;
    if ((rc = run_patchdown(h->down1, f1, B, S / 2, S / 2, C, 0, f2, s, "gemm_down1", next_dir(h)))) return rc;
    if ((rc = tap(h, "down1", f2, (size_t)B * (S / 2) * (S / 2) * 2 * C * 2, s))) return rc;
    if ((rc = run_stage(h, h->swin[1], f2, B, S / 2, 2 * C, s, "swin2"))) return rc;
    if (h->down2_split) {
        if ((rc = run_patchdown(h->down2, f2, B, S / 4, S / 4, 2 * C, 0, f3, s, "gemm_down2", next_dir(h)))) return rc;
    } else if ((rc = run_gemm(h->down2, f2, B, S / 2, S / 2, 2 * C, S / 4, S / 4, 2, 0, 0, 2, 0, 0, 0.f, nullptr, f3,
                              2 * C, 1, s, "gemm_down2", next_dir(h))))
        return rc;
    if (h->down2_split && (rc = run_gemm(h->down2b, f2, B, S / 2, S / 2, 2 * C, S / 4, S / 4, 2, 1, 0, 2, 0, 0, 0.f, f3, f3,
                                         2 * C, 1, s, "gemm_down2b", next_dir(h))))
        return rc;
    if ((rc = tap(h, "down2", f3, (size_t)B * (S / 4) * (S / 4) * 2 * C * 2, s))) return rc;
    if ((rc = run_stage(h, h->swin[2], f3, B, S / 4, 2 * C, s, "swin3"))) return rc;
    if ((rc = run_patchup(h->up2, f3, B, S / 4, S / 4, 2 * C, f2, s, "gemm_up2", next_dir(h)))) return rc;
    if ((rc = tap(h, "up2", f2, (size_t)B * (S / 2) * (S / 2) * 2 * C * 2, s))) return rc;
    if ((rc = run_stage(h, h->swin[3], f2, B, S / 2, 2 * C, s, "swin4"))) return rc;
    f16 *top = f1;
    if (h->has_proj2) {
        top = (f16 *)h->g1.p;
        if ((rc = run_linear(h->proj2, f1, B, S, S, 0, nullptr, top, s, "gemm_proj2", next_dir(h)))) return rc;
    }
    if ((rc = run_patchup(h->up1, f2, B, S / 2, S / 2, h->top_dim, top, s, "gemm_up1", next_dir(h)))) return rc;
    if ((rc = tap(h, "up1", top, (size_t)B * S * S * h->top_dim * 2, s))) return rc;
    if (h->top_dim == 96 && h->swin[4].back().fast && h->to_image_chained && !h->taps_on) {
        TailToImage ti;
        ti.w = h->to_image_chained; ti.bias = h->to_image.bias; ti.out = z; ti.H = S; ti.W = S; ti.ps = h->scale_factor;
        ti.n_real = h->to_image.n_real;
        return run_stage(h, h->swin[4], top, B, S, h->top_dim, s, "swin5", &ti);
    }
    if ((rc = run_stage(h, h->swin[4], top, B, S, h->top_dim, s, "swin5"))) return rc;
    if (h->scale_factor == 8) {
        f16 *pre = (f16 *)h->att.p;
        if ((rc = run_gemm(h->to_image_pre, top, B, S, S, h->top_dim, S, S, 1, 0, 0, 1, 0, 2, 0.2f, nullptr, pre, 192, 1, s,
                           "gemm_to_image_pre", next_dir(h))))
            return rc;
        top = pre;
    }
    if ((rc = run_gemm(h->to_image, top, B, S, S, h->top_dim, S, S, 1, 0, 0, 1, 2, 0, 0.f, nullptr, z, 0,
                       h->scale_factor, s, "gemm_to_image", next_dir(h))))
        return rc;
    return NUNIF_HIP_OK;
}

}
}

extern "C" int nunif_hip_swin_unet_create(const nunif_tensor_desc *tensors, int32_t n_tensors,
                                          int32_t scale_factor, nunif_swin_unet **handle) {
    NUNIF_REQUIRE(tensors && handle && n_tensors > 0, "swin_unet_create: NULL argument");
    NUNIF_REQUIRE(scale_factor == 1 || scale_factor == 2 || scale_factor == 4 || scale_factor == 8,
                  "swin_unet_create: scale_factor %d unsupported (1, 2, 4, 8)", scale_factor);
    const TensorMap m = tensor_map(tensors, n_tensors);
    nunif_swin_unet *h = new nunif_swin_unet();
    (void)hipGetDevice(&h->device);
    if (const char *v = getenv("NUNIF_BLOCK96")) h->block96 = atoi(v);
    if (const char *v = getenv("NUNIF_ATT_WM")) h->att_wm = atoi(v);
    h->gelu32 = scale_factor == 1;
    if (const char *v = getenv("NUNIF_SWIN_GELU32")) h->gelu32 = atoi(v);
    h->scale_factor = scale_factor;
    const std::string P = "unet.";
    int rc = NUNIF_HIP_OK;
    do {
        const HostTensor *w0, *b0, *w2, *b2;
        if ((rc = find(m, P + "patch.0.weight", &w0)) || (rc = find(m, P + "patch.0.bias", &b0)) ||
            (rc = find(m, P + "patch.2.weight", &w2)) || (rc = find(m, P + "patch.2.bias", &b2)))
            break;
        if (w2->shape.size() != 4 || w0->shape.size() != 4 || w0->shape[1] != 3) {
            set_error("patch conv: unexpected shape"); rc = NUNIF_HIP_EINVAL; break;
        }
        const int C = (int)w2->shape[0];
        const int C1 = (int)w0->shape[0];
        if (C % 96 != 0 || C1 * 2 != C) { set_error("base_dim %d unsupported", C); rc = NUNIF_HIP_EUNSUPPORTED; break; }
        h->C = C; h->heads = C / 16; h->C1 = C1; h->C1P = (C1 + 31) / 32 * 32;
        h->has_proj2 = scale_factor >= 4;
        h->top_dim = h->has_proj2 ? 2 * C : C;
        {
            std::vector<float> w(w0->data, w0->data + w0->numel), b(b0->data, b0->data + b0->numel);
            if ((rc = h->upload(w, &h->stem1_w)) || (rc = h->upload(b, &h->stem1_b))) break;
        }
        {
            const float *wd = w2->data;
            const int C1P = h->C1P;
            rc = make_linear(h, C, 9 * C1P, [=](int n, int k) {
                const int tap = k / C1P, ci = k % C1P;
                return ci < C1 ? wd[((size_t)n * C1 + ci) * 9 + tap] : 0.0f;
            }, b2->data, &h->stem2);
            if (rc) break;
        }
        if (stem_fused_supported(C1, C)) {
            const float *w0d = w0->data, *b0d = b0->data, *wd = w2->data;
            std::vector<f16> p1 = pack_nt_ks(C1, pad16(C1), 32, [=](int n, int k) {
                return k < 27 ? w0d[(size_t)n * 27 + k] : (k == 27 ? b0d[n] : 0.0f); });
            const int K2 = 448;
            std::vector<f16> stream = pack_ks_nt(C, C, K2, [=](int n, int k) {
                const int tap = k / C1, ci = k % C1;
                return k < 9 * C1 ? wd[((size_t)n * C1 + ci) * 9 + tap] : 0.0f; }, false, 0);
            if ((rc = h->upload(p1, &h->stemf_w1)) || (rc = h->upload(stream, &h->stemf_w2))) break;
        }
        if ((rc = make_stage(h, m, P + "swin1", C, 2, &h->swin[0]))) break;
        if ((rc = make_stage(h, m, P + "swin2", 2 * C, 2, &h->swin[1]))) break;
        if ((rc = make_stage(h, m, P + "swin3", 2 * C, 6, &h->swin[2]))) break;
        if ((rc = make_stage(h, m, P + "swin4", 2 * C, 2, &h->swin[3]))) break;
        if ((rc = make_stage(h, m, P + "swin5", h->top_dim, 2, &h->swin[4]))) break;
        auto make_down = [&](const std::string &key, int cin, int cout, Linear *L) -> int {
            const HostTensor *w, *b;
            int r;
            if ((r = find(m, key + ".conv.weight", &w)) || (r = find(m, key + ".conv.bias", &b))) return r;
            NUNIF_REQUIRE(w->numel == (int64_t)cout * cin * 4, "%s: shape", key.c_str());
            const float *wd = w->data;
            return make_linear(h, cout, 4 * cin, [=](int n, int k) {
                const int tap = k / cin, ci = k % cin;
                return wd[((size_t)n * cin + ci) * 4 + tap];
            }, b->data, L);
        };
        auto make_up = [&](const std::string &key, int cin, int cq, Linear *L) -> int {
            const HostTensor *w, *b;
            int r;
            if ((r = find(m, key + ".proj.weight", &w)) || (r = find(m, key + ".proj.bias", &b))) return r;
            NUNIF_REQUIRE(w->numel == (int64_t)4 * cq * cin, "%s: shape", key.c_str());
            const float *wd = w->data;
            std::vector<float> bb(4 * cq);
            for (int n = 0; n < 4 * cq; ++n) bb[n] = b->data[(n % cq) * 4 + n / cq];
            return make_linear(h, 4 * cq, cin, [=](int n, int k) {
                const int q = n / cq, c = n % cq;
                return wd[((size_t)(c * 4 + q)) * cin + k];
            }, bb.data(), L);
        };
        if ((rc = make_down(P + "down1", C, 2 * C, &h->down1))) break;
        {
            const HostTensor *w, *b;
            if ((rc = find(m, P + "down2.conv.weight", &w)) || (rc = find(m, P + "down2.conv.bias", &b))) break;
            const int cin = 2 * C, cout = 2 * C;
            if (w->numel != (int64_t)cout * cin * 4) { set_error("down2: shape"); rc = NUNIF_HIP_EINVAL; break; }
            const float *wd = w->data;
            std::vector<float> zero(cout, 0.0f);
            if ((rc = make_linear(h, cout, 2 * cin, [=](int n, int k) {
                    const int dx = k / cin, ci = k % cin; return wd[((size_t)n * cin + ci) * 4 + dx]; }, b->data, &h->down2)) ||
                (rc = make_linear(h, cout, 2 * cin, [=](int n, int k) {
                    const int dx = k / cin, ci = k % cin; return wd[((size_t)n * cin + ci) * 4 + 2 + dx]; }, zero.data(), &h->down2b)))
                break;
            h->down2_split = true;
        }
        if ((rc = make_up(P + "up2", 2 * C, 2 * C, &h->up2))) break;
        if ((rc = make_up(P + "up1", 2 * C, h->top_dim, &h->up1))) break;
        if (h->has_proj2 && (rc = make_plain_linear(h, m, P + "proj2", 2 * C, C, &h->proj2))) break;
        if (scale_factor == 8) {
            if ((rc = make_plain_linear(h, m, P + "to_image.proj.0", 192, h->top_dim, &h->to_image_pre)) ||
                (rc = make_plain_linear(h, m, P + "to_image.proj.2", 192, 192, &h->to_image)))
                break;
        } else if ((rc = make_plain_linear(h, m, P + "to_image.proj", 3 * scale_factor * scale_factor, h->top_dim,
                                           &h->to_image)))
            break;
        if (h->top_dim == 96 && 3 * scale_factor * scale_factor <= 16) {
            const HostTensor *tw;
            if ((rc = find(m, P + "to_image.proj.weight", &tw))) break;
            const float *wd = tw->data;
            const int nr = 3 * scale_factor * scale_factor, K = h->top_dim;
            std::vector<f16> ch = pack_nt_ks(nr, pad16(nr), K, [=](int n, int k) { return wd[(size_t)n * K + k]; }, true);
            if ((rc = h->upload(ch, &h->to_image_chained))) break;
        }
    } while (0);
    if (rc) {
        nunif_hip_swin_unet_destroy(h);
        return rc;
    }
    *handle = h;
    return NUNIF_HIP_OK;
}

extern "C" int nunif_hip_swin_unet_debug_taps(nunif_swin_unet *h, int32_t enable) {
    NUNIF_REQUIRE(h, "debug_taps: NULL handle");
    h->clear_taps();
    h->taps_on = enable != 0;
    return NUNIF_HIP_OK;
}

extern "C" int nunif_hip_swin_unet_get_tap(nunif_swin_unet *h, int32_t index, char *name, int32_t name_cap,
                                           void *host_dst, int64_t cap_bytes, int64_t *nbytes) {
    NUNIF_REQUIRE(h && nbytes, "get_tap: NULL argument");
    if (index < 0 || index >= (int)h->taps.size()) return 1;
    const auto &t = h->taps[index];
    if (name && name_cap > 0) { strncpy(name, t.name.c_str(), name_cap - 1); name[name_cap - 1] = 0; }
    *nbytes = (int64_t)t.bytes;
    if (host_dst) {
        NUNIF_REQUIRE(cap_bytes >= (int64_t)t.bytes, "get_tap: buffer too small");
        NUNIF_HIP_CHECK(hipDeviceSynchronize());
        NUNIF_HIP_CHECK(hipMemcpy(host_dst, t.dev, t.bytes, hipMemcpyDeviceToHost));
    }
    return NUNIF_HIP_OK;
}

extern "C" void nunif_hip_swin_unet_destroy(nunif_swin_unet *h) {
    if (!h) return;
    h->clear_taps();
    h->free_all();
    for (DeviceBuf *b : {&h->s1, &h->f1, &h->f2, &h->f3, &h->g1, &h->qkv, &h->att, &h->hid, &h->tile_out, &h->winmap[0], &h->winmap[1]}) b->release();
    delete h;
}

extern "C" int nunif_hip_swin_unet_forward(nunif_swin_unet *h, const float *x, float *z, int32_t batch,
                                           int32_t tile_size, void *stream) {
    NUNIF_REQUIRE(h && x && z && batch > 0, "swin_unet_forward: bad argument");
    return forward_impl(h, x, nullptr, nullptr, 0, z, batch, tile_size, (hipStream_t)stream);
}

extern "C" int nunif_hip_swin_unet_render(nunif_swin_unet *h, const float *x, float *y, int32_t x_h, int32_t x_w,
                                          int32_t tile_size, int32_t batch_size, void *stream) {
    NUNIF_REQUIRE(h && x && y && batch_size > 0, "swin_unet_render: bad argument");
    NUNIF_REQUIRE(h->scale_factor != 8, "swin_unet_render: the 8x net has no consistent tile geometry; use forward");
    const int s = h->scale_factor;
    nunif_tile_grid g;
    int rc = nunif_hip_tile_grid_init(x_h, x_w, s, 8 * s, tile_size, 4 * s, &g);
    if (rc) return rc;
    const int n_tiles = g.h_blocks * g.w_blocks;
    const size_t To = g.out_tile_size;
    if ((rc = h->tile_out.ensure((size_t)n_tiles * 3 * To * To * sizeof(float)))) return rc;
    float *tile_out = (float *)h->tile_out.p;
    hipStream_t st = (hipStream_t)stream;
    for (int t0 = 0; t0 < n_tiles; t0 += batch_size) {
        const int nb = std::min(batch_size, n_tiles - t0);
        if ((rc = forward_impl(h, nullptr, x, &g, t0, tile_out + (size_t)t0 * 3 * To * To, nb, tile_size, st)))
            return rc;
    }
    return launch_stitch(tile_out, y, &g, 3, st);
}

static int rows_grid(nunif_swin_unet *h, int32_t x_h, int32_t x_w, int32_t tile_size, nunif_tile_grid *g) {
    NUNIF_REQUIRE(h->scale_factor != 8, "swin_unet: the 8x net has no consistent tile geometry");
    const int s = h->scale_factor;
    int rc = nunif_hip_tile_grid_init(x_h, x_w, s, 8 * s, tile_size, 4 * s, g);
    if (rc) return rc;
    const size_t To = g->out_tile_size;
    return h->tile_out.ensure((size_t)g->h_blocks * g->w_blocks * 3 * To * To * sizeof(float));
}

extern "C" int nunif_hip_swin_unet_render_tile_rows(nunif_swin_unet *h, const float *x, int32_t x_h, int32_t x_w,
                                                    int32_t tile_size, int32_t batch_size, int32_t row_begin,
                                                    int32_t row_end, void *stream) {
    NUNIF_REQUIRE(h && x && batch_size > 0, "swin_unet_render_tile_rows: bad argument");
    nunif_tile_grid g;
    int rc = rows_grid(h, x_h, x_w, tile_size, &g);
    if (rc) return rc;
    NUNIF_REQUIRE(0 <= row_begin && row_begin <= row_end && row_end <= g.h_blocks, "tile rows [%d, %d) outside the grid of %d rows",
                  row_begin, row_end, g.h_blocks);
    const size_t To = g.out_tile_size;
    float *tile_out = (float *)h->tile_out.p;
    const int t_end = row_end * g.w_blocks;
    for (int t0 = row_begin * g.w_blocks; t0 < t_end; t0 += batch_size) {
        const int nb = std::min(batch_size, t_end - t0);
        if ((rc = forward_impl(h, nullptr, x, &g, t0, tile_out + (size_t)t0 * 3 * To * To, nb, tile_size, (hipStream_t)stream)))
            return rc;
    }
    return NUNIF_HIP_OK;
}

extern "C" int nunif_hip_swin_unet_tile_row_band(nunif_swin_unet *h, int32_t x_h, int32_t x_w, int32_t tile_size,
                                                 int32_t tile_row, int32_t row0, int32_t n_rows, float *band,
                                                 int32_t import_band, void *stream) {
    NUNIF_REQUIRE(h && band, "swin_unet_tile_row_band: bad argument");
    nunif_tile_grid g;
    int rc = rows_grid(h, x_h, x_w, tile_size, &g);
    if (rc) return rc;
    const int To = g.out_tile_size;
    NUNIF_REQUIRE(0 <= tile_row && tile_row < g.h_blocks && row0 >= 0 && n_rows > 0 && row0 + n_rows <= To, "tile_row_band: bad window");
    float *store = (float *)h->tile_out.p + (size_t)tile_row * g.w_blocks * 3 * To * To + (size_t)row0 * To;
    const size_t planes = (size_t)g.w_blocks * 3;
    if (import_band)
        NUNIF_HIP_CHECK(hipMemcpy2DAsync(store, (size_t)To * To * 4, band, (size_t)n_rows * To * 4, (size_t)n_rows * To * 4, planes,
                                         hipMemcpyDeviceToDevice, (hipStream_t)stream));
    else
        NUNIF_HIP_CHECK(hipMemcpy2DAsync(band, (size_t)n_rows * To * 4, store, (size_t)To * To * 4, (size_t)n_rows * To * 4, planes,
                                         hipMemcpyDeviceToDevice, (hipStream_t)stream));
    return NUNIF_HIP_OK;
}

extern "C" int nunif_hip_swin_unet_stitch_rows(nunif_swin_unet *h, float *y_band, int32_t x_h, int32_t x_w, int32_t tile_size,
                                               int32_t y_row_begin, int32_t y_row_end, void *stream) {
    NUNIF_REQUIRE(h && y_band, "swin_unet_stitch_rows: bad argument");
    nunif_tile_grid g;
    int rc = rows_grid(h, x_h, x_w, tile_size, &g);
    if (rc) return rc;
    return launch_stitch((const float *)h->tile_out.p, y_band, &g, 3, (hipStream_t)stream, y_row_begin, y_row_end - y_row_begin, 1);
}
```

Before: 323.7 MPix/s.

## Skip swin attention windows outside the image on edge tiles via cached window lists

For each tile batch, computes host-side which 6x6 attention windows of each full-resolution swin block can affect output pixels inside the image, tracing the extent back through shifted windows and the U-Net stages. It uploads compact window lists and per-list pixel maps, then runs qkv-attention and proj/MLP only on those windows. Plans are cached per grid and tile offset in an LRU list, with an event to synchronise across streams. This cuts wasted work on padded edge tiles, at the cost of plan-building overhead, extra device memory, and a risk of correctness errors if the extent analysis is wrong.

New measurement: 338.8 MPix/s, median of 6. +4.7%, better.

```diff
diff --git a/include/nunif_hip.h b/include/nunif_hip.h
--- a/include/nunif_hip.h
+++ b/include/nunif_hip.h
@@ -68,6 +68,13 @@
                                       void *stream);
 int nunif_hip_swin_unet_stitch_rows(nunif_swin_unet *handle, float *y_band, int32_t x_h, int32_t x_w, int32_t tile_size,
                                     int32_t y_row_begin, int32_t y_row_end, void *stream);
+
+typedef struct {
+    int32_t n_win[2];
+    int32_t wrap[2];
+} nunif_swin_block_extent;
+int nunif_hip_swin_unet_tile_extents(const nunif_tile_grid *grid, int32_t tile_index, const int32_t *blocks_per_stage,
+                                     const int32_t *shifts, int32_t to_image_fused, nunif_swin_block_extent *out);
 
 typedef struct nunif_swin_unet_v2 nunif_swin_unet_v2;
 int nunif_hip_swin_unet_v2_create(const nunif_tensor_desc *tensors, int32_t n_tensors, int32_t scale_factor,
diff --git a/nunif_amd/_hip.py b/nunif_amd/_hip.py
--- a/nunif_amd/_hip.py
+++ b/nunif_amd/_hip.py
@@ -26,6 +26,10 @@
                 "pad": (self.pad_l, self.pad_r, self.pad_t, self.pad_b),
                 "y_buffer_h": self.y_buffer_h, "y_buffer_w": self.y_buffer_w,
                 "input_tile_step": self.input_tile_step, "output_tile_step": self.output_tile_step}
+
+
+class SwinBlockExtent(ctypes.Structure):
+    _fields_ = [("n_win", c_int32 * 2), ("wrap", c_int32 * 2)]
 
 
 class TensorDesc(ctypes.Structure):
@@ -64,6 +68,8 @@
     "nunif_hip_swin_unet_render_tile_rows": (c_int32, [c_void_p, c_void_p, c_int32, c_int32, c_int32, c_int32, c_int32, c_int32, c_void_p]),
     "nunif_hip_swin_unet_tile_row_band": (c_int32, [c_void_p, c_int32, c_int32, c_int32, c_int32, c_int32, c_int32, c_void_p, c_int32, c_void_p]),
     "nunif_hip_swin_unet_stitch_rows": (c_int32, [c_void_p, c_void_p, c_int32, c_int32, c_int32, c_int32, c_int32, c_void_p]),
+    "nunif_hip_swin_unet_tile_extents": (c_int32, [ctypes.POINTER(TileGrid), c_int32, ctypes.POINTER(c_int32), ctypes.POINTER(c_int32),
+                                                   c_int32, ctypes.POINTER(SwinBlockExtent)]),
     "nunif_hip_swin_unet_v2_create": (c_int32, [ctypes.POINTER(TensorDesc), c_int32, c_int32, ctypes.POINTER(c_void_p)]),
     "nunif_hip_swin_unet_v2_destroy": (None, [c_void_p]),
     "nunif_hip_swin_unet_v2_forward": (c_int32, [c_void_p, c_void_p, c_void_p, c_int32, c_int32, c_int32, c_void_p]),
@@ -242,6 +248,17 @@
     return g
 
 
+def swin_tile_extents(grid, tile_index, blocks_per_stage=(2, 2, 6, 2, 2), shifts=None, to_image_fused=True):
+    n = sum(blocks_per_stage)
+    if shifts is None:
+        shifts = [3 if i % 2 else 0 for k in blocks_per_stage for i in range(k)]
+    per = (c_int32 * 5)(*blocks_per_stage)
+    sh = (c_int32 * n)(*shifts)
+    out = (SwinBlockExtent * n)()
+    check(lib().nunif_hip_swin_unet_tile_extents(ctypes.byref(grid), tile_index, per, sh, 1 if to_image_fused else 0, out))
+    return [(e.n_win[0], e.n_win[1], e.wrap[0], e.wrap[1]) for e in out]
+
+
 def blend_ramp(blend_size):
     buf = (c_float * max(1, blend_size))()
     check(lib().nunif_hip_blend_ramp(blend_size, buf))
diff --git a/nunif_amd/csrc/swin_block_tail.hip b/nunif_amd/csrc/swin_block_tail.hip
--- a/nunif_amd/csrc/swin_block_tail.hip
+++ b/nunif_amd/csrc/swin_block_tail.hip
@@ -264,6 +264,26 @@
     return NUNIF_HIP_OK;
 }
 
+__global__ void winmap_list_build_kernel(int *__restrict__ pixmap, const unsigned *__restrict__ list, int n_list, int H, int W, int shift) {
+    const int n = blockIdx.x * blockDim.x + threadIdx.x;
+    if (n >= 36 * n_list) return;
+    const int w = n / 36, t = n - 36 * w;
+    const unsigned e = list[w];
+    const int b = (int)(e >> 16), wy = (int)((e >> 8) & 255u), wx = (int)(e & 255u);
+    const int iy = t / 6, ix = t - 6 * iy;
+    int yy = wy * 6 + iy + shift, xx = wx * 6 + ix + shift;
+    if (yy >= H) yy -= H;
+    if (xx >= W) xx -= W;
+    pixmap[n] = (b * H + yy) * W + xx;
+}
+
+int launch_winmap_list_build(int *pixmap, const unsigned *win_list, int n_list, int H, int W, int shift, hipStream_t s) {
+    NUNIF_REQUIRE(pixmap && win_list && n_list > 0 && H % 6 == 0 && W % 6 == 0 && 36L * n_list < (1L << 31), "winmap: list of %d windows", n_list);
+    winmap_list_build_kernel<<<(unsigned)((36L * n_list + 255) / 256), 256, 0, s>>>(pixmap, win_list, n_list, H, W, shift);
+    NUNIF_LAUNCH_CHECK();
+    return NUNIF_HIP_OK;
+}
+
 constexpr int proj_mlp_stream_frags_c(int C) { return 2 * (C / 32) * (C / 32) + (2 * C / 32) * (2 * (C / 32) + C / 16); }
 
 int proj_mlp_stream_frags(int C) {
@@ -284,7 +304,7 @@
     WinMap wm;
     memset(&wm, 0, sizeof(wm));
     if (wmap) wm = *wmap;
-    NUNIF_REQUIRE(!wm.on || (wm.pixmap && wm.H % 6 == 0 && wm.W % 6 == 0 && M % ((long)wm.H * wm.W) == 0 && 96L * M < (1L << 31)),
+    NUNIF_REQUIRE(!wm.on || (wm.pixmap && wm.H % 6 == 0 && wm.W % 6 == 0 && M % 36 == 0 && 96L * M < (1L << 31)),
                   "proj_mlp: window map geometry");
     constexpr int MF = 2, WAVES = 8;
     auto go = [&](auto kern, int slot) -> int {
diff --git a/nunif_amd/csrc/swin_kernels.h b/nunif_amd/csrc/swin_kernels.h
--- a/nunif_amd/csrc/swin_kernels.h
+++ b/nunif_amd/csrc/swin_kernels.h
@@ -108,6 +108,7 @@
 struct TailToImage { const f16 *w; const float *bias; float *out; int H, W, ps, n_real; };
 struct WinMap { int on, H, W, shift; const int *pixmap; };
 int launch_winmap_build(int *pixmap, int B, int H, int W, int shift, hipStream_t s);
+int launch_winmap_list_build(int *pixmap, const unsigned *win_list, int n_list, int H, int W, int shift, hipStream_t s);
 int launch_proj_mlp(const f16 *att, f16 *x, const f16 *wstream, const float *bp, const float *b0, const float *b3,
                     long M, int C, hipStream_t s, const TailToImage *to_image = nullptr, int rev = 0,
                     const WinMap *wm = nullptr, int gelu32 = 0);
@@ -124,7 +125,8 @@
 
 constexpr int kQkvBiasFloatsPerHead = 36 * 52;
 int launch_qkv_attn_r(const f16 *x, f16 *att, const f16 *wres, const float *bqkv, const float *btab32,
-                      int B, int H, int W, int C, int heads, int shift, hipStream_t s, int rev = 0, int window_major = 0);
+                      int B, int H, int W, int C, int heads, int shift, hipStream_t s, int rev = 0, int window_major = 0,
+                      const unsigned *win_list = nullptr, int n_list = 0);
 
 int launch_window_attn(const f16 *qkv, f16 *out, const float *bias, int B, int H, int W, int heads, int hd,
                        int shift, hipStream_t s);
diff --git a/nunif_amd/csrc/swin_qkv_attn_r.hip b/nunif_amd/csrc/swin_qkv_attn_r.hip
--- a/nunif_amd/csrc/swin_qkv_attn_r.hip
+++ b/nunif_amd/csrc/swin_qkv_attn_r.hip
@@ -16,6 +16,7 @@
     const float *btab32;
     int B, H, W, shift, n_windows;
     int rev;
+    const unsigned *wlist;
 };
 
 __device__ __forceinline__ f16x4 mul4_to_f16(const f32x4 &o, float inv) {
@@ -116,10 +117,21 @@
             for (int ks = 0; ks < KS; ++ks) xf[mt][ks] = *reinterpret_cast<const f16x8 *>(xb + vo[mt] + 64 * ks);
         }
     };
-    auto decode = [&](int &wb, int &wy, int &wx, bool &special) {
-        wb = a.rev ? a.B - 1 - cb : cb;
-        wy = a.rev ? nwy - 1 - cy : cy;
-        wx = a.rev ? nwx - 1 - cx : cx;
+    auto list_slot = [&](int wi) {
+        const int i = wi < a.n_windows ? wi : a.n_windows - 1;
+        return a.rev ? a.n_windows - 1 - i : i;
+    };
+    int lslot = 0;
+    auto decode = [&](int wi, int &wb, int &wy, int &wx, bool &special) {
+        if (a.wlist) {
+            lslot = list_slot(wi);
+            const unsigned e = a.wlist[lslot];
+            wb = (int)(e >> 16); wy = (int)((e >> 8) & 255u); wx = (int)(e & 255u);
+        } else {
+            wb = a.rev ? a.B - 1 - cb : cb;
+            wy = a.rev ? nwy - 1 - cy : cy;
+            wx = a.rev ? nwx - 1 - cx : cx;
+        }
         special = a.shift > 0 && (wy == nwy - 1 || wx == nwx - 1);
     };
     auto advance = [&]() {
@@ -145,12 +157,12 @@
     f16x8 wnx = wl[lane];
     auto run_windows = [&]() {
     int wi = w0;
-    decode(wb, wy, wx, special);
-    auto step = [&]() { advance(); wi += wstride; decode(wb, wy, wx, special); };
+    decode(wi, wb, wy, wx, special);
+    auto step = [&]() { if (!a.wlist) advance(); wi += wstride; decode(wi, wb, wy, wx, special); };
     if (wi < a.n_windows) load_x(wb, wy, wx, special, xf, vo);
 #pragma unroll 1
     while (wi < a.n_windows) {
-        const int wq = (wb * nwy + wy) * nwx + wx;
+        const int wq = a.wlist ? lslot : (wb * nwy + wy) * nwx + wx;
         char *ab = reinterpret_cast<char *>(a.att) + (WM ? (long)wq * (HEADS * 36 * HD * 2) : (long)wb * img_bytes);
         const unsigned wm_base = (unsigned)__builtin_amdgcn_readfirstlane((unsigned)wq * (unsigned)(HEADS * 36 * HD * 2));
 
@@ -307,19 +319,23 @@
 }
 
 int launch_qkv_attn_r(const f16 *x, f16 *att, const f16 *wres, const float *bqkv, const float *btab32,
-                      int B, int H, int W, int C, int heads, int shift, hipStream_t s, int rev, int window_major) {
+                      int B, int H, int W, int C, int heads, int shift, hipStream_t s, int rev, int window_major,
+                      const unsigned *win_list, int n_list) {
     NUNIF_REQUIRE(H % 6 == 0 && W % 6 == 0, "qkv_attn: %dx%d not a multiple of the 6x6 window", H, W);
     NUNIF_REQUIRE(heads == 6 && (C == 96 || C == 192), "qkv_attn: C=%d heads=%d unsupported", C, heads);
     if (H <= 6) shift = 0;
     QkvAttnRArgs a;
     a.x = x; a.att = att; a.wres = wres; a.bqkv = bqkv; a.btab32 = btab32;
     a.B = B; a.H = H; a.W = W; a.shift = shift;
-    a.n_windows = B * (H / 6) * (W / 6);
+    NUNIF_REQUIRE(!win_list || (window_major && n_list > 0 && n_list <= B * (H / 6) * (W / 6) && B < 65536 && H / 6 < 256 && W / 6 < 256),
+                  "qkv_attn: a window list needs the window-major map and at most 65535 x 255 x 255 windows");
+    a.n_windows = win_list ? n_list : B * (H / 6) * (W / 6);
+    a.wlist = win_list;
     a.rev = rev;
     NUNIF_REQUIRE(!window_major || C == 96, "qkv_attn: the window-major att map exists for C = 96 only");
     NUNIF_REQUIRE(!window_major || (long)a.n_windows * (6 * 36 * 16 * 2) < (1L << 32),
                   "qkv_attn: the window-major att map of %d windows does not fit 32-bit byte offsets", a.n_windows);
-    const double tok = (double)B * H * W;
+    const double tok = 36.0 * a.n_windows;
     const int kWavesR = C == 96 ? 16 : 8;
     const int wgs = (a.n_windows + kWavesR - 1) / kWavesR;
     int grid = wgs < 256 ? wgs : 256;
diff --git a/nunif_amd/csrc/swin_unet.cpp b/nunif_amd/csrc/swin_unet.cpp
--- a/nunif_amd/csrc/swin_unet.cpp
+++ b/nunif_amd/csrc/swin_unet.cpp
@@ -2,6 +2,7 @@
 #include <cmath>
 #include <cstdlib>
 #include <cstring>
+#include <list>
 #include <string>
 #include <vector>
 
@@ -36,10 +37,76 @@
     float *b96_btab = nullptr;
 };
 
+struct SkipBlock {
+    unsigned *list = nullptr;
+    int *pixmap = nullptr;
+    int n_windows = 0;
+};
+
+struct SkipPlan {
+    nunif_tile_grid grid = {};
+    int tile_begin = 0, B = 0;
+    std::vector<SkipBlock> stage[5];
+    void *dev = nullptr;
+    size_t bytes = 0;
+    std::vector<unsigned> host;
+    hipStream_t built_on = nullptr;
+    hipEvent_t ready = nullptr;
+};
+
+int block_extent_back(int e, int S, int shift, int32_t *n_win, int32_t *wrap) {
+    const int nw = S / 6;
+    if (S <= 6) shift = 0;
+    if (shift == 0) {
+        *n_win = std::min(nw, (e + 5) / 6);
+        *wrap = 0;
+        return std::min(S, 6 * *n_win);
+    }
+    *n_win = std::min(nw - 1, (std::max(e - 3, 0) + 5) / 6);
+    *wrap = 1;
+    return *n_win == nw - 1 ? S : 3 + 6 * *n_win;
+}
+
 }
 }
 
 using namespace nunif;
+
+extern "C" int nunif_hip_swin_unet_tile_extents(const nunif_tile_grid *g, int32_t tile_index, const int32_t *blocks_per_stage,
+                                                const int32_t *shifts, int32_t to_image_fused, nunif_swin_block_extent *out) {
+    (void)to_image_fused;
+    NUNIF_REQUIRE(g && blocks_per_stage && shifts && out, "tile_extents: NULL argument");
+    NUNIF_REQUIRE(tile_index >= 0 && tile_index < g->h_blocks * g->w_blocks, "tile_extents: tile %d outside the grid", tile_index);
+    const int S = g->tile_size - 16;
+    NUNIF_REQUIRE(S > 0 && S % 24 == 0 && g->scale > 0 && g->out_tile_size == S * g->scale,
+                  "tile_extents: the grid is not a swin_unet grid (tile %d, output tile %d)", g->tile_size, g->out_tile_size);
+    int first[6] = {0};
+    for (int st = 0; st < 5; ++st) {
+        NUNIF_REQUIRE(blocks_per_stage[st] >= 0, "tile_extents: negative block count");
+        first[st + 1] = first[st] + blocks_per_stage[st];
+    }
+    const int size[5] = {S, S / 2, S / 4, S / 2, S};
+    const int ti[2] = {tile_index / g->w_blocks, tile_index % g->w_blocks};
+    const int y_len[2] = {g->y_h, g->y_w};
+    for (int ax = 0; ax < 2; ++ax) {
+        const int n_px = std::min(g->out_tile_size, y_len[ax] - g->output_tile_step * ti[ax]);
+        auto stage_back = [&](int st, int e) {
+            for (int i = blocks_per_stage[st] - 1; i >= 0; --i) {
+                nunif_swin_block_extent &o = out[first[st] + i];
+                if (e <= 0) { o.n_win[ax] = 0; o.wrap[ax] = 0; continue; }
+                e = block_extent_back(e, size[st], shifts[first[st] + i], &o.n_win[ax], &o.wrap[ax]);
+            }
+            return std::max(e, 0);
+        };
+        const int e5 = n_px <= 0 ? 0 : std::min(S, (n_px + g->scale - 1) / g->scale);
+        const int top_in = stage_back(4, e5);
+        const int e4_in = stage_back(3, (top_in + 1) / 2);
+        const int e3_in = stage_back(2, (e4_in + 1) / 2);
+        const int e2_in = stage_back(1, std::min(size[1], std::max(2 * e3_in, e4_in)));
+        (void)stage_back(0, std::min(size[0], std::max(2 * e2_in, top_in)));
+    }
+    return NUNIF_HIP_OK;
+}
 
 struct nunif_swin_unet : DeviceOwner {
     int scale_factor = 2;
@@ -61,6 +128,19 @@
     DeviceBuf s1, f1, f2, f3, g1, qkv, att, hid, tile_out;
     DeviceBuf winmap[2];
     int winmap_B = 0, winmap_S = 0;
+    std::list<SkipPlan> plans;
+    size_t plan_bytes = 0;
+    const SkipPlan *plan = nullptr;
+    void drop_plan(std::list<SkipPlan>::iterator it) {
+        if (it->ready) (void)hipEventDestroy(it->ready);
+        (void)hipFree(it->dev);
+        plan_bytes -= it->bytes;
+        plans.erase(it);
+    }
+    void clear_plans() {
+        while (!plans.empty()) drop_plan(plans.begin());
+        plan = nullptr;
+    }
     int device = 0;
     struct Tap { std::string name; void *dev; size_t bytes; };
     bool taps_on = false;
@@ -280,7 +360,7 @@
 }
 
 int run_stage(nunif_swin_unet *h, std::vector<Block> &blocks, f16 *x, int B, int S, int dim, hipStream_t s,
-              const char *name, const TailToImage *to_image = nullptr) {
+              const char *name, const TailToImage *to_image = nullptr, const std::vector<SkipBlock> *skip = nullptr) {
     f16 *qkv = (f16 *)h->qkv.p, *att = (f16 *)h->att.p;
     const size_t tok = (size_t)B * S * S;
     int rc;
@@ -319,8 +399,9 @@
             continue;
         }
         const bool att_wm = dim == 96 && h->att_wm && !h->taps_on && 96L * (long)tok < (1L << 31);
+        const SkipBlock *sk = skip && att_wm && i < skip->size() && (*skip)[i].list ? &(*skip)[i] : nullptr;
         if ((rc = launch_qkv_attn_r(x, att, bl.qkv_res, bl.qkv_rbias, bl.attn_btab32, B, S, S, dim, h->heads, shift, s, next_dir(h),
-                                    att_wm ? 1 : 0)))
+                                    att_wm ? 1 : 0, sk ? sk->list : nullptr, sk ? sk->n_windows : 0)))
             return rc;
         if ((rc = tap(h, tn + ".attn", att, tok * dim * 2, s))) return rc;
         const bool last = i + 1 == blocks.size();
@@ -330,7 +411,9 @@
         } else {
             const int eff_shift = S <= 6 ? 0 : shift;
             WinMap wmap = {att_wm ? 1 : 0, S, S, eff_shift, nullptr};
-            if (att_wm) {
+            if (sk) {
+                wmap.pixmap = sk->pixmap;
+            } else if (att_wm) {
                 if (h->winmap_S != S || B > h->winmap_B) {
                     for (int k = 0; k < 2; ++k) {
                         if ((rc = h->winmap[k].ensure(tok * sizeof(int)))) return rc;
@@ -340,7 +423,7 @@
                 }
                 wmap.pixmap = (const int *)h->winmap[eff_shift ? 1 : 0].p;
             }
-            if ((rc = launch_proj_mlp(att, x, bl.tail_stream, bl.proj.bias, bl.mlp0.bias, bl.mlp3.bias, (long)tok, dim, s,
+            if ((rc = launch_proj_mlp(att, x, bl.tail_stream, bl.proj.bias, bl.mlp0.bias, bl.mlp3.bias, sk ? 36L * sk->n_windows : (long)tok, dim, s,
                                       last ? to_image : nullptr, next_dir(h), &wmap, h->gelu32)))
                 return rc;
         }
@@ -367,12 +450,97 @@
     return NUNIF_HIP_OK;
 }
 
+constexpr size_t kMaxPlans = 1024, kMaxPlanBytes = (size_t)1 << 30;
+
+int skip_plan(nunif_swin_unet *h, const nunif_tile_grid *g, int t0, int B, hipStream_t s, const SkipPlan **out) {
+    *out = nullptr;
+    const int S = g->tile_size - 16, nw = S / 6;
+    if (!h->att_wm || h->taps_on || h->block96 || S <= 6 || nw >= 256 || B >= 65536 || 96L * B * S * S >= (1L << 31) ||
+        g->out_tile_size != S * g->scale)
+        return NUNIF_HIP_OK;
+    for (auto it = h->plans.begin(); it != h->plans.end(); ++it)
+        if (it->tile_begin == t0 && it->B == B && memcmp(g, &it->grid, sizeof(*g)) == 0) {
+            h->plans.splice(h->plans.begin(), h->plans, it);
+            if (it->dev && it->built_on != s) NUNIF_HIP_CHECK(hipStreamWaitEvent(s, it->ready, 0));
+            *out = &*it;
+            return NUNIF_HIP_OK;
+        }
+    int32_t per_stage[5], n_blocks = 0;
+    std::vector<int32_t> shifts;
+    for (int st = 0; st < 5; ++st) {
+        per_stage[st] = (int32_t)h->swin[st].size();
+        for (int i = 0; i < per_stage[st]; ++i) shifts.push_back(i % 2 == 1 ? 3 : 0);
+        n_blocks += per_stage[st];
+    }
+    std::vector<std::vector<nunif_swin_block_extent>> ext(B, std::vector<nunif_swin_block_extent>(n_blocks));
+    int rc;
+    for (int b = 0; b < B; ++b)
+        if ((rc = nunif_hip_swin_unet_tile_extents(g, t0 + b, per_stage, shifts.data(), 0, ext[b].data()))) return rc;
+    h->plans.emplace_front();
+    SkipPlan &plan = h->plans.front();
+    plan.grid = *g; plan.tile_begin = t0; plan.B = B; plan.built_on = s;
+    struct Piece { int st, i, shift; size_t first, n; };
+    std::vector<Piece> pieces;
+    int first = 0;
+    for (int st = 0; st < 5; first += per_stage[st], ++st) {
+        const int dim = st == 0 ? h->C : (st == 4 ? h->top_dim : 2 * h->C);
+        bool fast = (st == 0 || st == 4) && dim == 96;
+        for (const Block &bl : h->swin[st]) fast = fast && bl.fast;
+        if (!fast) continue;
+        plan.stage[st].resize(per_stage[st]);
+        for (int i = 0; i < per_stage[st]; ++i) {
+            const size_t at = plan.host.size();
+            for (int b = 0; b < B; ++b) {
+                const nunif_swin_block_extent &e = ext[b][first + i];
+                auto active = [&](int ax, int w) { return w < e.n_win[ax] || (e.wrap[ax] && w == nw - 1); };
+                for (int wy = 0; wy < nw; ++wy) {
+                    if (!active(0, wy)) continue;
+                    for (int wx = 0; wx < nw; ++wx)
+                        if (active(1, wx)) plan.host.push_back((unsigned)b << 16 | (unsigned)wy << 8 | (unsigned)wx);
+                }
+            }
+            const size_t n = plan.host.size() - at;
+            if (n == (size_t)B * nw * nw || n == 0) { plan.host.resize(at); continue; }
+            pieces.push_back({st, i, shifts[first + i], at, n});
+        }
+    }
+    if (pieces.empty()) { *out = &plan; return NUNIF_HIP_OK; }
+    const size_t list_bytes = (plan.host.size() * 4 + 255) / 256 * 256;
+    plan.bytes = list_bytes + plan.host.size() * 36 * 4;
+    auto fail = [&](int code) { h->drop_plan(h->plans.begin()); return code; };
+    if (hipMalloc(&plan.dev, plan.bytes) != hipSuccess) {
+        set_error("hipMalloc(%zu) of the window lists failed", plan.bytes);
+        plan.bytes = 0;
+        return fail(NUNIF_HIP_ENOMEM);
+    }
+    h->plan_bytes += plan.bytes;
+    if (hipMemcpyAsync(plan.dev, plan.host.data(), plan.host.size() * 4, hipMemcpyHostToDevice, s) != hipSuccess ||
+        hipEventCreateWithFlags(&plan.ready, hipEventDisableTiming) != hipSuccess) {
+        set_error("upload of the window lists failed");
+        return fail(NUNIF_HIP_EHIP);
+    }
+    for (const Piece &pc : pieces) {
+        SkipBlock &sb = plan.stage[pc.st][pc.i];
+        sb.list = (unsigned *)plan.dev + pc.first;
+        sb.pixmap = (int *)((char *)plan.dev + list_bytes) + pc.first * 36;
+        sb.n_windows = (int)pc.n;
+        if ((rc = launch_winmap_list_build(sb.pixmap, sb.list, sb.n_windows, S, S, pc.shift, s))) return fail(rc);
+    }
+    if (hipEventRecord(plan.ready, s) != hipSuccess) { set_error("hipEventRecord failed"); return fail(NUNIF_HIP_EHIP); }
+    while (h->plans.size() > kMaxPlans || (h->plan_bytes > kMaxPlanBytes && h->plans.size() > 1)) h->drop_plan(std::prev(h->plans.end()));
+    *out = &plan;
+    return NUNIF_HIP_OK;
+}
+
 int forward_impl(nunif_swin_unet *h, const float *x, const float *frame, const nunif_tile_grid *grid,
-                 int tile_begin, float *z, int B, int T, hipStream_t s) {
+                 int tile_begin, float *z, int B, int T, hipStream_t s, bool skip_pad = false) {
     const int S = T - 16, C = h->C;
     NUNIF_REQUIRE(T > 16 && S % 12 == 0 && S % 16 == 0, "tile_size %d is not valid for swin_unet", T);
     int rc;
     if ((rc = ensure_workspace(h, B, T))) return rc;
+    h->plan = nullptr;
+    if (frame && skip_pad && (rc = skip_plan(h, grid, tile_begin, B, s, &h->plan))) return rc;
+    auto skip_of = [&](int st) { return h->plan && !h->plan->stage[st].empty() ? &h->plan->stage[st] : nullptr; };
     f16 *s1 = (f16 *)h->s1.p, *f1 = (f16 *)h->f1.p, *f2 = (f16 *)h->f2.p, *f3 = (f16 *)h->f3.p;
 
     if (h->stemf_w2 && stem_fused_supported(h->C1, (int)C)) {
@@ -406,7 +574,7 @@
         return rc;
 stem_done:
     if ((rc = tap(h, "stem", f1, (size_t)B * S * S * C * 2, s))) return rc;
-    if ((rc = run_stage(h, h->swin[0], f1, B, S, C, s, "swin1"))) return rc;
+    if ((rc = run_stage(h, h->swin[0], f1, B, S, C, s, "swin1", nullptr, skip_of(0)))) return rc;
     if ((rc = run_patchdown(h->down1, f1, B, S / 2, S / 2, C, 0, f2, s, "gemm_down1", next_dir(h)))) return rc;
     if ((rc = tap(h, "down1", f2, (size_t)B * (S / 2) * (S / 2) * 2 * C * 2, s))) return rc;
     if ((rc = run_stage(h, h->swin[1], f2, B, S / 2, 2 * C, s, "swin2"))) return rc;
@@ -434,9 +602,9 @@
         TailToImage ti;
         ti.w = h->to_image_chained; ti.bias = h->to_image.bias; ti.out = z; ti.H = S; ti.W = S; ti.ps = h->scale_factor;
         ti.n_real = h->to_image.n_real;
-        return run_stage(h, h->swin[4], top, B, S, h->top_dim, s, "swin5", &ti);
-    }
-    if ((rc = run_stage(h, h->swin[4], top, B, S, h->top_dim, s, "swin5"))) return rc;
+        return run_stage(h, h->swin[4], top, B, S, h->top_dim, s, "swin5", &ti, skip_of(4));
+    }
+    if ((rc = run_stage(h, h->swin[4], top, B, S, h->top_dim, s, "swin5", nullptr, skip_of(4)))) return rc;
     if (h->scale_factor == 8) {
         f16 *pre = (f16 *)h->att.p;
         if ((rc = run_gemm(h->to_image_pre, top, B, S, S, h->top_dim, S, S, 1, 0, 0, 1, 0, 2, 0.2f, nullptr, pre, 192, 1, s,
@@ -601,6 +769,7 @@
 extern "C" void nunif_hip_swin_unet_destroy(nunif_swin_unet *h) {
     if (!h) return;
     h->clear_taps();
+    h->clear_plans();
     h->free_all();
     for (DeviceBuf *b : {&h->s1, &h->f1, &h->f2, &h->f3, &h->g1, &h->qkv, &h->att, &h->hid, &h->tile_out, &h->winmap[0], &h->winmap[1]}) b->release();
     delete h;
@@ -610,6 +779,11 @@
                                            int32_t tile_size, void *stream) {
     NUNIF_REQUIRE(h && x && z && batch > 0, "swin_unet_forward: bad argument");
     return forward_impl(h, x, nullptr, nullptr, 0, z, batch, tile_size, (hipStream_t)stream);
+}
+
+static bool skip_pad_enabled() {
+    const char *v = getenv("NUNIF_SWIN_SKIP_PAD");
+    return !(v && atoi(v) == 0);
 }
 
 extern "C" int nunif_hip_swin_unet_render(nunif_swin_unet *h, const float *x, float *y, int32_t x_h, int32_t x_w,
@@ -625,9 +799,10 @@
     if ((rc = h->tile_out.ensure((size_t)n_tiles * 3 * To * To * sizeof(float)))) return rc;
     float *tile_out = (float *)h->tile_out.p;
     hipStream_t st = (hipStream_t)stream;
+    const bool skip_pad = skip_pad_enabled();
     for (int t0 = 0; t0 < n_tiles; t0 += batch_size) {
         const int nb = std::min(batch_size, n_tiles - t0);
-        if ((rc = forward_impl(h, nullptr, x, &g, t0, tile_out + (size_t)t0 * 3 * To * To, nb, tile_size, st)))
+        if ((rc = forward_impl(h, nullptr, x, &g, t0, tile_out + (size_t)t0 * 3 * To * To, nb, tile_size, st, skip_pad)))
             return rc;
     }
     return launch_stitch(tile_out, y, &g, 3, st);
@@ -654,9 +829,10 @@
     const size_t To = g.out_tile_size;
     float *tile_out = (float *)h->tile_out.p;
     const int t_end = row_end * g.w_blocks;
+    const bool skip_pad = skip_pad_enabled();
     for (int t0 = row_begin * g.w_blocks; t0 < t_end; t0 += batch_size) {
         const int nb = std::min(batch_size, t_end - t0);
-        if ((rc = forward_impl(h, nullptr, x, &g, t0, tile_out + (size_t)t0 * 3 * To * To, nb, tile_size, (hipStream_t)stream)))
+        if ((rc = forward_impl(h, nullptr, x, &g, t0, tile_out + (size_t)t0 * 3 * To * To, nb, tile_size, (hipStream_t)stream, skip_pad)))
             return rc;
     }
     return NUNIF_HIP_OK;
```
